# XuyangBai/D3Feat

Hardware: AMD Instinct MI355X
Metric: fragments/sec (30k-pt clouds) (higher is better)
Workload: dtype f32; 1 GPU; SURVEY §8d config #2: synthetic 3DMatch room fragment, 300k raw pts -> grid subsample 0.03 m (~29k pts per cloud) -> self-pair -> 5-level pyramid -> full KPFCNN forward (random-init weights (reference initialiser, seed 42), 14.1M params)...; points_per_cloud=29369, fragments_per_gpu=2141, parallelism=fragment-dp1, fragments_per_replay=12, engine_fallbacks=0, engine_isolated_replays=0

## Files before the change

### d3feat_amd/csrc/grid_subsample.hip

```cpp
#include <cstdlib>
#include "prims.h"
#include "radix_sort.h"

#define GS_EMPTY 0xFFFFFFFFFFFFFFFFull
#define GS_KEYBITS 56
#define GS_KEYMASK ((1ull << GS_KEYBITS) - 1ull)
#define GS_MAX_PROBE 4096

__constant__ unsigned long long D3F_CHAIN_DEV[D3F_NCHAIN] = {
    13ull, 29ull, 59ull, 127ull, 257ull, 541ull, 1109ull, 2357ull, 5087ull, 10273ull, 20753ull, 42043ull, 85229ull,
    172933ull, 351061ull, 712697ull, 1447153ull, 2938679ull, 5967347ull, 12117689ull, 24607243ull, 49969847ull,
    101473717ull, 206062531ull, 418451333ull, 849749479ull, 1725587117ull, 3504151727ull};

struct GsElem {
    float org[3];
    int pad0;
    unsigned long long NX, NY, NZ;
    long long bbase;
};

static unsigned long long gs_chain_ge(long long n) {
    for (int j = 0; j < D3F_NCHAIN; ++j)
        if ((long long)D3F_CHAIN_HOST[j] >= n) return D3F_CHAIN_HOST[j];
    return D3F_CHAIN_HOST[D3F_NCHAIN - 1];
}

__device__ __forceinline__ unsigned long long gs_mix(unsigned long long x) {
    x ^= x >> 33; x *= 0xff51afd7ed558ccdull; x ^= x >> 33; x *= 0xc4ceb9fe1a85ec53ull; x ^= x >> 33;
    return x;
}

__device__ __forceinline__ int gs_bits(unsigned long long x) {
    int b = 0;
    while (x) { ++b; x >>= 1; }
    return b;
}
__device__ __forceinline__ void gs_prep(const unsigned* __restrict__ bbox, const int* __restrict__ offs, int B, float dl,
                                        GsElem* __restrict__ el, int* __restrict__ status, RsMeta* __restrict__ smeta,
                                        int n_cap) {
    __shared__ unsigned long long sCells[256];
    const int b = threadIdx.x;
    unsigned long long cells = 0ull;
    if (b < B) {
        GsElem e;
        e.pad0 = 0;
        const int len = offs[b + 1] - offs[b];
        if (len <= 0) {
            atomicOr(&status[1], D3F_ST_EMPTY_ELEMENT);
            e.org[0] = e.org[1] = e.org[2] = 0.f;
            e.NX = e.NY = e.NZ = 1;
        } else {
            const float inv = __fdiv_rn(1.0f, dl);
            float mx[3];
#pragma unroll
            for (int d = 0; d < 3; ++d) {
                float mn = d3f_ord2f(__hip_atomic_load(&bbox[b * 6 + d], __ATOMIC_RELAXED, __HIP_MEMORY_SCOPE_AGENT));
                mx[d] = d3f_ord2f(__hip_atomic_load(&bbox[b * 6 + 3 + d], __ATOMIC_RELAXED, __HIP_MEMORY_SCOPE_AGENT));
                e.org[d] = __fmul_rn(floorf(__fmul_rn(mn, inv)), dl);
            }
            e.NX = (unsigned long long)fmaxf(floorf(__fdiv_rn(__fsub_rn(mx[0], e.org[0]), dl)), 0.f) + 1ull;
            e.NY = (unsigned long long)fmaxf(floorf(__fdiv_rn(__fsub_rn(mx[1], e.org[1]), dl)), 0.f) + 1ull;
            e.NZ = (unsigned long long)fmaxf(floorf(__fdiv_rn(__fsub_rn(mx[2], e.org[2]), dl)), 0.f) + 1ull;
        }
        long long base = 0;
        for (int j = 0; j < b; ++j) {
            long long l = offs[j + 1] - offs[j];
            unsigned long long nb = D3F_CHAIN_DEV[D3F_NCHAIN - 1];
            for (int c = 0; c < D3F_NCHAIN; ++c)
                if ((long long)D3F_CHAIN_DEV[c] >= l) { nb = D3F_CHAIN_DEV[c]; break; }
            base += (long long)nb;
        }
        e.bbase = base;
        el[b] = e;
        const double c = (double)e.NX * (double)e.NY * (double)e.NZ;
        cells = c >= 1.8e19 ? 0xFFFFFFFFFFFFFFFFull : e.NX * e.NY * e.NZ;
    }
    if (!smeta) return;
    sCells[threadIdx.x] = cells;
    __syncthreads();
    if (threadIdx.x == 0) {
        unsigned long long mx = 1ull;
        for (int j = 0; j < B; ++j) mx = sCells[j] > mx ? sCells[j] : mx;
        int kb = gs_bits(mx - 1ull);
        if (kb < 1) kb = 1;
        const int eb = gs_bits((unsigned long long)(B - 1));
        RsMeta m;
        m.n = min(offs[B], n_cap);
        m.kb = kb;
        m.bits = kb + eb;
        if (m.bits > 32) {
            atomicOr(&status[1], D3F_ST_KEY_WIDTH);
            m.n = 0;
            m.bits = 8;
        }
        m.npass = (m.bits + 7) / 8;
        *smeta = m;
    }
}
struct GsPrepEpi {
    const unsigned* bbox; const int* offs; int B; float dl; GsElem* el; int* status; RsMeta* smeta; int n_cap;
    __device__ __forceinline__ void operator()() const { gs_prep(bbox, offs, B, dl, el, status, smeta, n_cap); }
};

__global__ void __launch_bounds__(256) gs_insert_kernel(const float* __restrict__ pts, int N, const int* __restrict__ offs,
                                                        int B, float dl, const GsElem* __restrict__ el,
                                                        unsigned long long* __restrict__ tkey, unsigned* __restrict__ tfirst,
                                                        unsigned long long capmask, int* __restrict__ slot,
                                                        int* __restrict__ status) {
    const int i = blockIdx.x * blockDim.x + threadIdx.x;
    if (i >= min(N, offs[B])) return;
    const int b = d3f_find_elem(offs, B, i);
    const GsElem e = el[b];
    const float fx = floorf(__fdiv_rn(__fsub_rn(pts[3 * (size_t)i + 0], e.org[0]), dl));
    const float fy = floorf(__fdiv_rn(__fsub_rn(pts[3 * (size_t)i + 1], e.org[1]), dl));
    const float fz = floorf(__fdiv_rn(__fsub_rn(pts[3 * (size_t)i + 2], e.org[2]), dl));
    int st = 0;
    if (fx < 0.f || fy < 0.f || fz < 0.f) st |= D3F_ST_NEG_CELL;
    const unsigned long long ix = (unsigned long long)fmaxf(fx, 0.f), iy = (unsigned long long)fmaxf(fy, 0.f),
                             iz = (unsigned long long)fmaxf(fz, 0.f);
    const unsigned long long key = ix + e.NX * iy + e.NX * e.NY * iz;
    if (key > GS_KEYMASK) st |= D3F_ST_KEY_RANGE;
    if (st) atomicOr(&status[1], st);
    const unsigned long long word = ((unsigned long long)b << GS_KEYBITS) | (key & GS_KEYMASK);
    unsigned long long h = gs_mix(word) & capmask;
    bool placed = false;
    for (int probe = 0; probe < GS_MAX_PROBE; ++probe) {
        unsigned long long prev = atomicCAS(&tkey[h], GS_EMPTY, word);
        if (prev == GS_EMPTY || prev == word) { placed = true; break; }
        h = (h + 1) & capmask;
    }
    if (!placed) atomicOr(&status[1], D3F_ST_OUT_OVERFLOW);
    atomicMin(&tfirst[h], (unsigned)i);
    slot[i] = (int)h;
}

struct GsMarkIn {
    const int* n_dev; const int* slot; const unsigned* tfirst;
    __device__ __forceinline__ int operator()(int i) const { return (i < *n_dev && tfirst[slot[i]] == (unsigned)i) ? 1 : 0; }
};

__global__ void __launch_bounds__(256) gs_chain_kernel(int N, const int* __restrict__ slot, const unsigned* __restrict__ tfirst,
                                                       const unsigned long long* __restrict__ tkey,
                                                       const int* __restrict__ vscan, const int* __restrict__ vbase,
                                                       int* __restrict__ pvid,
                                                       unsigned long long* __restrict__ vkey, int* __restrict__ vhead,
                                                       int* __restrict__ vcnt, int* __restrict__ pnext,
                                                       const int* __restrict__ n_dev) {
    const int i = blockIdx.x * blockDim.x + threadIdx.x;
    if (i >= min(N, *n_dev)) return;
    const int s = slot[i];
    const int fi = (int)tfirst[s];
    const int v = d3f_scan_at(vscan, vbase, fi);
    pvid[i] = v;
    if (fi == i) vkey[v] = tkey[s] & GS_KEYMASK;
    pnext[i] = atomicExch(&vhead[v], i);
    atomicAdd(&vcnt[v], 1);
}

struct GsRankScan {
    const int* vscan; const int* vbase;
    __device__ __forceinline__ int operator()(int p) const { return d3f_scan_at(vscan, vbase, p); }
};
struct GsRankBits {
    const unsigned* fbits; const int* wscan; const int* wbase;
    __device__ __forceinline__ int operator()(int p) const {
        const int w = p >> 5;
        return d3f_scan_at(wscan, wbase, w) + __popc(fbits[w] & ((1u << (p & 31)) - 1u));
    }
};
template <class Rank>
struct GsMoffsEpi {
    const int* offs; int B; Rank rank; int* meta; int* moffs; int* sub_lens; int* status_dev;
    int out_cap;
    int elem_cap;
    __device__ __forceinline__ void operator()(int M) const {
        if (threadIdx.x != 0) return;
        meta[0] = M;
        const int N = offs[B];
        for (int b = 0; b <= B; ++b) moffs[b] = (b == B || offs[b] >= N) ? M : rank(offs[b]);
        bool over = M > out_cap ||
                    (__hip_atomic_load(&meta[1], __ATOMIC_RELAXED, __HIP_MEMORY_SCOPE_AGENT) & (D3F_ST_OUT_OVERFLOW | D3F_ST_KEY_WIDTH));
        for (int b = 0; b < B; ++b) over = over || (moffs[b + 1] - moffs[b] > elem_cap);
        if (over && !(__hip_atomic_load(&meta[1], __ATOMIC_RELAXED, __HIP_MEMORY_SCOPE_AGENT) & D3F_ST_KEY_WIDTH))
            atomicOr(&meta[1], D3F_ST_OUT_OVERFLOW);
        for (int b = 0; b < B; ++b) {
            const int l = over ? 0 : moffs[b + 1] - moffs[b];
            meta[2 + b] = l;
            sub_lens[b] = l;
        }
        if (status_dev) {
            status_dev[0] = over ? 0 : M;
            status_dev[1] = __hip_atomic_load(&meta[1], __ATOMIC_RELAXED, __HIP_MEMORY_SCOPE_AGENT);
        }
    }
};

__global__ void __launch_bounds__(256) gs_rank_kernel(int N, const int* __restrict__ n_dev, const int* __restrict__ pvid,
                                                      const int* __restrict__ vhead, const int* __restrict__ pnext,
                                                      const int* __restrict__ vstart, const int* __restrict__ sbase,
                                                      int* __restrict__ sorted) {
    const int i = blockIdx.x * blockDim.x + threadIdx.x;
    if (i >= min(N, *n_dev)) return;
    const int v = pvid[i];
    int r = 0;
    for (int j = vhead[v]; j >= 0; j = pnext[j]) r += (j < i) ? 1 : 0;
    sorted[d3f_scan_at(vstart, sbase, v) + r] = i;
}

__device__ __forceinline__ int gs_ld(const int* p) {
    return __hip_atomic_load(p, __ATOMIC_RELAXED, __HIP_MEMORY_SCOPE_AGENT);
}

__device__ __forceinline__ int gs_mod(unsigned long long key, unsigned nb, double inv_nb) {
    const unsigned long long q = (unsigned long long)((double)key * inv_nb);
    long long r = (long long)(key - q * (unsigned long long)nb);
    r += (r < 0) ? (long long)nb : 0;
    r += (r < 0) ? (long long)nb : 0;
    r -= (r >= (long long)nb) ? (long long)nb : 0;
    r -= (r >= (long long)nb) ? (long long)nb : 0;
    return (int)r;
}

#define GS_SMALL_LAST 6
#define GS_TILE 1024

struct GsOrderArgs {
    const unsigned long long* vkey;
    const int* moffs;
    const int* offs;
    const GsElem* el;
    int* P[2];
    int* nx[2];
    int* cd;
    int* bkt[2];
    int* bf[2];
    int* bc[2];
    int* bh[2];
    int* tsum;
    int* vpos;
    int max_m;
};

#define GS_SMALL_NB 1109
#define GS_SMALL_T 256
__global__ void __launch_bounds__(GS_SMALL_T) gs_order_small_kernel(GsOrderArgs A, int small_last) {
    __shared__ int wsum[GS_SMALL_T / 64];
    __shared__ int sBF[GS_SMALL_NB], sBC[GS_SMALL_NB], sBH[GS_SMALL_NB], sNX[GS_SMALL_NB], sCD[GS_SMALL_NB], sBK[GS_SMALL_NB];
    __shared__ int sL[2][GS_SMALL_NB];
    __shared__ unsigned long long sKey[GS_SMALL_NB];
    const int b = blockIdx.x;
    const int tid = threadIdx.x, lane = tid & 63, w = tid >> 6;
    const int M = A.moffs[b + 1] - A.moffs[b];
    if (M <= 0) return;
    const unsigned long long* key = A.vkey + A.moffs[b];
    int* VP = A.vpos + A.moffs[b];
    const long long bbase = A.el[b].bbase;
    if (small_last > GS_SMALL_LAST) small_last = GS_SMALL_LAST;
    for (int t = tid; t < min(M, GS_SMALL_NB); t += GS_SMALL_T) sKey[t] = key[t];
    int lo = 0, cur = 0;
    bool done = false;
    __syncthreads();
    for (int j = 0; j <= small_last && j < D3F_NCHAIN; ++j) {
        const int nb = (int)D3F_CHAIN_DEV[j];
        const double inv_nb = 1.0 / (double)nb;
        const bool last = M <= nb;
        const int hi = last ? M : nb;
        const int* La = sL[cur];
        int* Lb = sL[cur ^ 1];
        for (int t = tid; t < nb; t += GS_SMALL_T) { sBF[t] = 0x7fffffff; sBC[t] = 0; sBH[t] = -1; }
        __syncthreads();
        for (int t = tid; t < hi; t += GS_SMALL_T) {
            const int id = (t < lo) ? La[t] : t;
            const int bk = gs_mod(sKey[id], (unsigned)nb, inv_nb);
            atomicMin(&sBF[bk], t);
            atomicAdd(&sBC[bk], 1);
            sNX[t] = atomicExch(&sBH[bk], t);
            sBK[t] = bk;
        }
        __syncthreads();
        int carry = 0;
        for (int c0 = 0; c0 < hi; c0 += GS_SMALL_T) {
            const int u = c0 + tid, t = hi - 1 - u;
            int c = 0;
            if (u < hi) {
                const int bk = sBK[t];
                c = (sBF[bk] == t) ? sBC[bk] : 0;
            }
            int x = c;
#pragma unroll
            for (int d = 1; d < 64; d <<= 1) {
                int y = __shfl_up(x, d, 64);
                if (lane >= d) x += y;
            }
            if (lane == 63) wsum[w] = x;
            __syncthreads();
            int wbase = 0, tot = 0;
#pragma unroll
            for (int q = 0; q < GS_SMALL_T / 64; ++q) {
                int v = wsum[q];
                if (q < w) wbase += v;
                tot += v;
            }
            __syncthreads();
            if (u < hi) sCD[t] = carry + wbase + x - c;
            carry += tot;
        }
        __syncthreads();
        for (int t = tid; t < hi; t += GS_SMALL_T) {
            const int id = (t < lo) ? La[t] : t;
            const int bk = sBK[t];
            int r = 0;
            for (int q = sBH[bk]; q >= 0; q = sNX[q]) r += (q > t) ? 1 : 0;
            const int dest = sCD[sBF[bk]] + r;
            Lb[dest] = id;
            if (last) VP[id] = dest;
        }
        __syncthreads();
        cur ^= 1;
        if (last) { done = true; break; }
        lo = hi;
    }
    if (!done && small_last + 1 < D3F_NCHAIN) {
        const int j = small_last + 1;
        int* P = A.P[j & 1] + A.offs[b];
        for (int t = tid; t < lo; t += GS_SMALL_T) P[t] = sL[cur][t];
        const int nb = (int)D3F_CHAIN_DEV[j];
        int* BF = A.bf[j & 1] + bbase;
        int* BC = A.bc[j & 1] + bbase;
        int* BH = A.bh[j & 1] + bbase;
        for (int t = tid; t < nb; t += GS_SMALL_T) { BF[t] = 0x7fffffff; BC[t] = 0; BH[t] = -1; }
    }
}

__device__ __forceinline__ bool gs_round(const GsOrderArgs& A, int b, int j, int& M, int& lo, int& hi, int& nb, bool& last) {
    M = A.moffs[b + 1] - A.moffs[b];
    lo = (int)D3F_CHAIN_DEV[j - 1];
    if (M <= lo || M > A.max_m) return false;
    nb = (int)D3F_CHAIN_DEV[j];
    last = M <= nb;
    hi = last ? M : nb;
    return true;
}

__global__ void __launch_bounds__(256) gs_order_insert_kernel(GsOrderArgs A, int j) {
    const int b = blockIdx.y;
    int M, lo, hi, nb;
    bool last;
    if (!gs_round(A, b, j, M, lo, hi, nb, last)) return;
    const int t = blockIdx.x * 256 + threadIdx.x;
    if (t >= hi) return;
    const int o = A.offs[b];
    const long long bbase = A.el[b].bbase;
    const int id = (t < lo) ? A.P[j & 1][o + t] : t;
    const int bk = gs_mod(A.vkey[A.moffs[b] + id], (unsigned)nb, 1.0 / (double)nb);
    atomicMin(&A.bf[j & 1][bbase + bk], t);
    atomicAdd(&A.bc[j & 1][bbase + bk], 1);
    A.nx[j & 1][o + t] = atomicExch(&A.bh[j & 1][bbase + bk], t);
    A.bkt[j & 1][o + t] = bk;
}

__device__ __forceinline__ void gs_order_scan_sums(const GsOrderArgs& A, int j, int b, int* wsum) {
    int M, lo, hi, nb;
    bool last;
    if (!gs_round(A, b, j, M, lo, hi, nb, last)) return;
    int* ts = A.tsum + A.offs[b] / GS_TILE + b;
    const int ntiles = (hi + GS_TILE - 1) / GS_TILE;
    const int tid = threadIdx.x, lane = tid & 63, w = tid >> 6;
    int carry = 0;
    for (int c0 = 0; c0 < ntiles; c0 += 256) {
        const int i = c0 + tid;
        const int v = (i < ntiles) ? __hip_atomic_load(&ts[i], __ATOMIC_RELAXED, __HIP_MEMORY_SCOPE_AGENT) : 0;
        int x = v;
#pragma unroll
        for (int d = 1; d < 64; d <<= 1) {
            int y = __shfl_up(x, d, 64);
            if (lane >= d) x += y;
        }
        if (lane == 63) wsum[w] = x;
        __syncthreads();
        int wbase = 0, tot = 0;
#pragma unroll
        for (int q = 0; q < 4; ++q) {
            int s = wsum[q];
            if (q < w) wbase += s;
            tot += s;
        }
        __syncthreads();
        if (i < ntiles) ts[i] = carry + wbase + x - v;
        carry += tot;
    }
}

__global__ void __launch_bounds__(256) gs_order_scan_tiles_kernel(GsOrderArgs A, int j, int B, unsigned* __restrict__ counter) {
    __shared__ int wsum[4];
    const int b = blockIdx.y;
    int M, lo, hi, nb;
    bool last;
    const int tile = blockIdx.x;
    const bool active = gs_round(A, b, j, M, lo, hi, nb, last) && tile * GS_TILE < hi;
    if (!active) return;
    {
        const int o = A.offs[b];
        const long long bbase = A.el[b].bbase;
        const int tid = threadIdx.x, lane = tid & 63, w = tid >> 6;
        if (!last && j + 1 < D3F_NCHAIN) {
            const int nbn = (int)D3F_CHAIN_DEV[j + 1];
            const int stride = ((hi + GS_TILE - 1) / GS_TILE) * 256;
            for (int i = tile * 256 + tid; i < nbn; i += stride) {
                A.bf[(j + 1) & 1][bbase + i] = 0x7fffffff;
                A.bc[(j + 1) & 1][bbase + i] = 0;
                A.bh[(j + 1) & 1][bbase + i] = -1;
            }
        }
        int c[4], s = 0;
#pragma unroll
        for (int k = 0; k < 4; ++k) {
            const int u = tile * GS_TILE + tid * 4 + k, t = hi - 1 - u;
            c[k] = 0;
            if (u < hi) {
                const int bk = A.bkt[j & 1][o + t];
                c[k] = (A.bf[j & 1][bbase + bk] == t) ? A.bc[j & 1][bbase + bk] : 0;
            }
            s += c[k];
        }
        int x = s;
#pragma unroll
        for (int d = 1; d < 64; d <<= 1) {
            int y = __shfl_up(x, d, 64);
            if (lane >= d) x += y;
        }
        if (lane == 63) wsum[w] = x;
        __syncthreads();
        int wbase = 0, tot = 0;
#pragma unroll
        for (int q = 0; q < 4; ++q) {
            int v = wsum[q];
            if (q < w) wbase += v;
            tot += v;
        }
        int run = wbase + x - s;
#pragma unroll
        for (int k = 0; k < 4; ++k) {
            const int u = tile * GS_TILE + tid * 4 + k;
            if (u < hi) A.cd[o + hi - 1 - u] = run;
            run += c[k];
        }
        if (tid == 0) A.tsum[o / GS_TILE + b + tile] = tot;
    }
    if (!d3f_last_block(counter + b, (unsigned)((hi + GS_TILE - 1) / GS_TILE))) return;
    gs_order_scan_sums(A, j, b, wsum);
}

__global__ void __launch_bounds__(256) gs_order_place_kernel(GsOrderArgs A, int j) {
    const int b = blockIdx.y;
    int M, lo, hi, nb;
    bool last;
    if (!gs_round(A, b, j, M, lo, hi, nb, last)) return;
    const int t = blockIdx.x * 256 + threadIdx.x;
    const int o = A.offs[b];
    const long long bbase = A.el[b].bbase;
    const bool next = !last && j + 1 < D3F_NCHAIN;
    const int nbn = next ? (int)D3F_CHAIN_DEV[j + 1] : 1;
    int id = -1, pos = -1;
    if (t < hi) {
        id = (t < lo) ? A.P[j & 1][o + t] : t;
        const int bk = A.bkt[j & 1][o + t];
        int r = 0;
        for (int q = A.bh[j & 1][bbase + bk]; q >= 0; q = A.nx[j & 1][o + q]) r += (q > t) ? 1 : 0;
        const int f = A.bf[j & 1][bbase + bk];
        const int dest = A.cd[o + f] + A.tsum[o / GS_TILE + b + (hi - 1 - f) / GS_TILE] + r;
        A.P[(j + 1) & 1][o + dest] = id;
        if (last) A.vpos[A.moffs[b] + id] = dest;
        pos = dest;
    } else if (next && t < min(M, nbn)) {
        id = pos = t;
    }
    if (next && id >= 0) {
        const int bk = gs_mod(A.vkey[A.moffs[b] + id], (unsigned)nbn, 1.0 / (double)nbn);
        atomicMin(&A.bf[(j + 1) & 1][bbase + bk], pos);
        atomicAdd(&A.bc[(j + 1) & 1][bbase + bk], 1);
        A.nx[(j + 1) & 1][o + pos] = atomicExch(&A.bh[(j + 1) & 1][bbase + bk], pos);
        A.bkt[(j + 1) & 1][o + pos] = bk;
    }
}

#include "gs_small.h"

__global__ void __launch_bounds__(RS_THREADS) gs_sortkey_kernel(const float* __restrict__ pts, const float* const* __restrict__ ptrs,
                                                                const int* __restrict__ offs, int B,
                                                                float dl, const GsElem* __restrict__ el,
                                                                const RsMeta* __restrict__ smeta, unsigned* __restrict__ skey,
                                                                unsigned* __restrict__ hist, int* __restrict__ status) {
    __shared__ unsigned sHist[256];
    __shared__ int sOffs[D3F_MAX_BATCH + 1];
    __shared__ GsElem sEl[D3F_MAX_BATCH];
    __shared__ const float* sBase[D3F_MAX_BATCH];
    const int n = smeta->n, kb = smeta->kb;
    const int tile = blockIdx.x;
    if ((long long)tile * RS_TILE >= (long long)n) return;
    for (int t = threadIdx.x; t <= B; t += RS_THREADS) sOffs[t] = offs[t];
    for (int t = threadIdx.x; t < B; t += RS_THREADS) {
        sEl[t] = el[t];
        sBase[t] = ptrs ? ptrs[t] - 3 * (size_t)offs[t] : pts;
    }
    __syncthreads();
    const int w = threadIdx.x >> 6, lane = threadIdx.x & 63;
    const int base = tile * RS_TILE + w * RS_WAVE_ITEMS + lane;
    const int wlo = tile * RS_TILE + w * RS_WAVE_ITEMS, whi = min(wlo + RS_WAVE_ITEMS, n) - 1;
    int b0 = 0;
    while (b0 + 1 < B && wlo >= sOffs[b0 + 1]) ++b0;
    const bool one_cloud = (b0 + 1 >= B) || whi < sOffs[b0 + 1];
    unsigned key[RS_ROUNDS], vm = 0u;
    int st = 0;
#pragma unroll
    for (int r = 0; r < RS_ROUNDS; ++r) {
        const int i = base + r * 64;
        key[r] = 0u;
        if (i < n) {
            int b = b0;
            if (!one_cloud)
                while (b + 1 < B && i >= sOffs[b + 1]) ++b;
            const float ox = sEl[b].org[0], oy = sEl[b].org[1], oz = sEl[b].org[2];
            const unsigned NX = (unsigned)sEl[b].NX, NY = (unsigned)sEl[b].NY;
            const float* __restrict__ P = sBase[b];
            const float fx = floorf(__fdiv_rn(__fsub_rn(P[3 * (size_t)i + 0], ox), dl));
            const float fy = floorf(__fdiv_rn(__fsub_rn(P[3 * (size_t)i + 1], oy), dl));
            const float fz = floorf(__fdiv_rn(__fsub_rn(P[3 * (size_t)i + 2], oz), dl));
            if (fx < 0.f || fy < 0.f || fz < 0.f) st |= D3F_ST_NEG_CELL;
            const unsigned ix = (unsigned)fmaxf(fx, 0.f), iy = (unsigned)fmaxf(fy, 0.f), iz = (unsigned)fmaxf(fz, 0.f);
            const unsigned k = ix + NX * (iy + NY * iz);
            key[r] = (kb < 32 ? ((unsigned)b << kb) : 0u) | (kb < 32 ? (k & ((1u << kb) - 1u)) : k);
            skey[i] = key[r];
            vm |= 1u << r;
        }
    }
    if (st) atomicOr(&status[1], st);
    rs_tile_histogram(key, vm, 0, sHist, hist + (size_t)tile * 256);
}

__global__ void __launch_bounds__(256) gs_heads_kernel(int N, const RsMeta* __restrict__ smeta, const unsigned* __restrict__ key0,
                                                       const unsigned* __restrict__ key1, const unsigned* __restrict__ val0,
                                                       const unsigned* __restrict__ val1, unsigned* __restrict__ fbits) {
    const int j = blockIdx.x * blockDim.x + threadIdx.x;
    if (j >= min(N, smeta->n)) return;
    const unsigned* __restrict__ ks = (smeta->npass & 1) ? key1 : key0;
    const unsigned* __restrict__ vs = (smeta->npass & 1) ? val1 : val0;
    const unsigned k = ks[j];
    if (j == 0 || ks[j - 1] != k) {
        const unsigned i = vs[j];
        atomicOr(&fbits[i >> 5], 1u << (i & 31u));
    }
}
struct GsBitsIn {
    const unsigned* fbits;
    __device__ __forceinline__ int operator()(int w) const { return __popc(fbits[w]); }
};
__global__ void __launch_bounds__(256) gs_runs_kernel(int N, const RsMeta* __restrict__ smeta, const unsigned* __restrict__ key0,
                                                      const unsigned* __restrict__ key1, const unsigned* __restrict__ val0,
                                                      const unsigned* __restrict__ val1, GsRankBits rank,
                                                      const float* __restrict__ pts, const float* const* __restrict__ ptrs,
                                                      const int* __restrict__ offs, unsigned long long* __restrict__ vkey,
                                                      float* __restrict__ bary) {
    __shared__ float sx[256], sy[256], sz[256];
    __shared__ unsigned sk[256];
    const int n = min(N, smeta->n);
    const int j0 = blockIdx.x * 256;
    if (j0 >= n) return;
    const int t = threadIdx.x, j = j0 + t;
    const unsigned* __restrict__ ks = (smeta->npass & 1) ? key1 : key0;
    const unsigned* __restrict__ vs = (smeta->npass & 1) ? val1 : val0;
    unsigned k = 0u, pi = 0u, kprev = 0u;
    float px = 0.f, py = 0.f, pz = 0.f;
    if (j < n) {
        k = ks[j];
        pi = vs[j];
        kprev = j > 0 ? ks[j - 1] : 0u;
        if (ptrs) {
            const int b = smeta->kb < 32 ? (int)(k >> smeta->kb) : 0;
            pts = ptrs[b] - 3 * (size_t)offs[b];
        }
        px = pts[3 * (size_t)pi + 0]; py = pts[3 * (size_t)pi + 1]; pz = pts[3 * (size_t)pi + 2];
    }
    sx[t] = px; sy[t] = py; sz[t] = pz;
    sk[t] = k;
    __syncthreads();
    if (j >= n || (j != 0 && kprev == k)) return;
    const int v = rank((int)pi);
    float ax = px, ay = py, az = pz;
    int c = 1;
    const int lim = min(256, n - j0);
    while (t + c < lim && sk[t + c] == k) {
        ax = __fadd_rn(ax, sx[t + c]);
        ay = __fadd_rn(ay, sy[t + c]);
        az = __fadd_rn(az, sz[t + c]);
        ++c;
    }
    if (t + c == 256) {
        while (j + c < n && ks[j + c] == k) {
            const size_t q = vs[j + c];
            ax = __fadd_rn(ax, pts[3 * q + 0]);
            ay = __fadd_rn(ay, pts[3 * q + 1]);
            az = __fadd_rn(az, pts[3 * q + 2]);
            ++c;
        }
    }
    const float sc = (float)(1.0 / (double)c);
    vkey[v] = (unsigned long long)(smeta->kb < 32 ? (k & ((1u << smeta->kb) - 1u)) : k);
    bary[3 * (size_t)v + 0] = __fmul_rn(ax, sc);
    bary[3 * (size_t)v + 1] = __fmul_rn(ay, sc);
    bary[3 * (size_t)v + 2] = __fmul_rn(az, sc);
}
__global__ void __launch_bounds__(256) gs_emit_kernel(int* __restrict__ status, const int* __restrict__ moffs, int B,
                                                      const int* __restrict__ vpos, const float* __restrict__ bary,
                                                      float* __restrict__ out_p, int out_cap) {
    const int v = blockIdx.x * blockDim.x + threadIdx.x;
    if (v >= status[0]) return;
    const int b = d3f_find_elem(moffs, B, v);
    const size_t dest = (size_t)moffs[b] + (size_t)vpos[v];
    if (dest >= (size_t)out_cap) {
        atomicOr(&status[1], D3F_ST_OUT_OVERFLOW);
        return;
    }
    out_p[3 * dest + 0] = bary[3 * (size_t)v + 0];
    out_p[3 * dest + 1] = bary[3 * (size_t)v + 1];
    out_p[3 * dest + 2] = bary[3 * (size_t)v + 2];
}


__global__ void __launch_bounds__(256) gs_accum_kernel(const float* __restrict__ pts, const float* __restrict__ feat,
                                                       int fdim, int* __restrict__ status,
                                                       const int* __restrict__ moffs, int B,
                                                       const int* __restrict__ vstart, const int* __restrict__ sbase,
                                                       const int* __restrict__ vcnt,
                                                       const int* __restrict__ sorted, const int* __restrict__ vpos,
                                                       float* __restrict__ out_p, float* __restrict__ out_f, int out_cap) {
    const int v = blockIdx.x * blockDim.x + threadIdx.x;
    if (v >= status[0]) return;
    const int b = d3f_find_elem(moffs, B, v);
    const int n = vcnt[v], st = sbase ? d3f_scan_at(vstart, sbase, v) : vstart[v];
    const size_t dest = (size_t)moffs[b] + (size_t)vpos[v];
    if (dest >= (size_t)out_cap) {
        atomicOr(&status[1], D3F_ST_OUT_OVERFLOW);
        return;
    }
    float sx = 0.f, sy = 0.f, sz = 0.f;
    for (int t = 0; t < n; ++t) {
        const size_t i = (size_t)sorted[st + t];
        sx = __fadd_rn(sx, pts[3 * i + 0]);
        sy = __fadd_rn(sy, pts[3 * i + 1]);
        sz = __fadd_rn(sz, pts[3 * i + 2]);
    }
    const float sc = (float)(1.0 / (double)n);
    out_p[3 * dest + 0] = __fmul_rn(sx, sc);
    out_p[3 * dest + 1] = __fmul_rn(sy, sc);
    out_p[3 * dest + 2] = __fmul_rn(sz, sc);
    if (fdim > 0) {
        const float cf = (float)n;
        for (int f = 0; f < fdim; ++f) {
            float s = 0.f;
            for (int t = 0; t < n; ++t) s = __fadd_rn(s, feat[(size_t)sorted[st + t] * fdim + f]);
            out_f[dest * fdim + f] = __fdiv_rn(s, cf);
        }
    }
}

__global__ void __launch_bounds__(256) gs_fill_kernel(int* __restrict__ p, size_t n, int v) {
    const size_t i = (size_t)blockIdx.x * blockDim.x + threadIdx.x;
    if (i < n) p[i] = v;
}
__global__ void __launch_bounds__(256) gs_labels_kernel(int N, int ldim, const int* __restrict__ cls,
                                                        const int* __restrict__ pvid, const int* __restrict__ moffs, int B,
                                                        const int* __restrict__ vpos, int* __restrict__ out_c) {
    const int i = blockIdx.x * blockDim.x + threadIdx.x;
    if (i >= N) return;
    const int v = pvid[i];
    const int b = d3f_find_elem(moffs, B, v);
    const size_t dest = (size_t)moffs[b] + (size_t)vpos[v];
    for (int l = 0; l < ldim; ++l) atomicMax(&out_c[dest * ldim + l], cls[(size_t)i * ldim + l]);
}

struct GsLayout {
    size_t cap;
    long long bucket_total;
};
static GsLayout gs_layout(int N, int B, int keys = -1) {
    GsLayout L;
    L.cap = 64;
    const size_t nk = (size_t)((keys > 0 && keys < N) ? keys : (N > 0 ? N : 1));
    while (L.cap < (size_t)2 * nk) L.cap <<= 1;
    L.bucket_total = (long long)(2.24 * (double)N) + 16ll * B + 64;
    return L;
}

extern "C" size_t d3f_grid_subsample_workspace_bytes(int N, int B, int fdim, int ldim) {
    (void)fdim; (void)ldim;
    if (N < 0 || B < 1) return 0;
    GsLayout L = gs_layout(N, B);
    size_t n = (size_t)(N > 0 ? N : 1);
    size_t bytes = 0;
    bytes += d3f_align((B + 1) * sizeof(int)) * 2 + d3f_align((B + 2) * sizeof(int));
    bytes += d3f_align(B * 6 * sizeof(unsigned));
    bytes += d3f_align(B * sizeof(GsElem));
    bytes += d3f_align(L.cap * sizeof(unsigned long long));
    bytes += d3f_align(L.cap * sizeof(int));
    bytes += d3f_align(n * sizeof(unsigned long long));
    bytes += 16 * d3f_align(n * sizeof(int));
    bytes += 6 * d3f_align((size_t)L.bucket_total * sizeof(int));
    bytes += d3f_align((n / GS_TILE + B + 8) * sizeof(int));
    bytes += 2 * d3f_align(d3f_scan_base_ints(N) * sizeof(int)) + d3f_align((4 + D3F_NCHAIN * (size_t)B) * sizeof(unsigned));
    bytes += d3f_align(rs_hist_words(N) * sizeof(unsigned)) + d3f_align((n / 32 + 2) * sizeof(unsigned)) +
             d3f_align(3 * n * sizeof(float)) + d3f_align(sizeof(RsMeta));
    bytes += d3f_align(7 * (size_t)B * (n < 16384 ? n : 16384) * sizeof(float)) + 256 + 2 * d3f_align(B * sizeof(int));
    return bytes + 4096;
}

template <int T, int R>
static int gs_small_launch(const GsSmallArgs& A, float* sub_points, int* sub_lens_dev, int* status_dev, hipStream_t stream) {
    static std::atomic<unsigned long long> lds_done{0ull};
    const void* const fns[] = {(const void*)gs_small_kernel<T, R>};
    if (d3f_opt_in_lds(lds_done, fns, (int)gss_lds_bytes<T, R>(GSS_NB_MAX)) != D3F_OK) return D3F_ERR_HIP;
    gs_small_kernel<T, R><<<A.B, T, gss_lds_bytes<T, R>(A.nbmax), stream>>>(A);
    D3F_LAUNCH_CHECK();
    gs_small_pack_kernel<<<d3f_cdiv(A.out_cap, 256), 256, 0, stream>>>(A, sub_points, sub_lens_dev, status_dev);
    D3F_LAUNCH_CHECK();
    return D3F_OK;
}
static int gs_run_small(const float* points, int N, const int* lens_dev, int B, float dl, float* sub_points, int M_cap, int elem_cap,
                        int pc, int* sub_lens_dev, int* status_dev, void* workspace, size_t workspace_bytes, hipStream_t stream) {
    if (elem_cap <= 0 || elem_cap > M_cap) elem_cap = M_cap;
    if (elem_cap > pc) elem_cap = pc;
    D3fArena ar(workspace, workspace_bytes);
    GsSmallArgs A;
    A.stage = ar.take<float>(3 * (size_t)B * (size_t)elem_cap);
    A.recs = ar.take<float>(4 * (size_t)B * (size_t)elem_cap);
    A.mcount = ar.take<int>(B);
    A.cflags = ar.take<int>(B);
    if (!ar.ok) return D3F_ERR_WORKSPACE;
    A.pts = points; A.lens = lens_dev; A.B = B; A.dl = dl; A.elem_cap = elem_cap; A.out_cap = M_cap;
    A.nbmax = GSS_NB_MAX;
    for (int j = 0; j < D3F_NCHAIN; ++j)
        if ((long long)D3F_CHAIN_HOST[j] >= (long long)elem_cap) { A.nbmax = (int)D3F_CHAIN_HOST[j]; break; }
    if (A.nbmax > GSS_NB_MAX) A.nbmax = GSS_NB_MAX;
    if (A.nbmax < 1109) A.nbmax = 1109;
    if (pc <= 2048) return gs_small_launch<256, 8>(A, sub_points, sub_lens_dev, status_dev, stream);
    if (pc <= 4096) return gs_small_launch<512, 8>(A, sub_points, sub_lens_dev, status_dev, stream);
    if (pc <= 8192) return gs_small_launch<1024, 8>(A, sub_points, sub_lens_dev, status_dev, stream);
    if (pc <= 12288) return gs_small_launch<1024, 12>(A, sub_points, sub_lens_dev, status_dev, stream);
    return gs_small_launch<1024, 16>(A, sub_points, sub_lens_dev, status_dev, stream);
}

static int gs_run(const float* points, int N, const int* lens_dev, int B, float dl, const float* features, int fdim,
                  const int* classes, int ldim, float* sub_points, int M_cap, int elem_cap, int elem_points, float* sub_features,
                  int* sub_classes, int* sub_lens_dev, int* status_host, int* status_dev, void* workspace,
                  size_t workspace_bytes, hipStream_t stream, const float* const* ptrs = nullptr) {
    const bool async = status_dev != nullptr;
    if (async && !features && ldim == 0 && !ptrs) {
        const int pc = (elem_points > 0 && elem_points < N) ? elem_points : N;
        int ec = (elem_cap > 0 && elem_cap < M_cap) ? elem_cap : M_cap;
        if (ec > pc) ec = pc;
        if (pc <= 16384 && ec <= GSS_NB_MAX) return gs_run_small(points, N, lens_dev, B, dl, sub_points, M_cap, elem_cap, pc, sub_lens_dev, status_dev,
                                             workspace, workspace_bytes, stream);
    }
    GsLayout L = gs_layout(N, B, async ? M_cap : -1);
    D3fArena ar(workspace, workspace_bytes);
    const size_t n = (size_t)N;
    int* offs = ar.take<int>(B + 1);
    int* moffs = ar.take<int>(B + 1);
    unsigned* bbox = ar.take<unsigned>(B * 6);
    GsElem* el = ar.take<GsElem>(B);
    const int ncounters = 4 + D3F_NCHAIN * B;
    unsigned* counters = ar.take<unsigned>(ncounters);
    unsigned long long* tkey = ar.take<unsigned long long>(L.cap);
    unsigned* tfirst = ar.take<unsigned>(L.cap);
    int* vhead = ar.take<int>(n);
    int* meta = ar.take<int>(B + 2);
    int* vcnt = ar.take<int>(n);
    unsigned long long* vkey = ar.take<unsigned long long>(n);
    int* slot = ar.take<int>(n);
    int* vscan = ar.take<int>(n);
    int* pvid = ar.take<int>(n);
    int* pnext = ar.take<int>(n);
    int* vstart = ar.take<int>(n);
    int* sorted = ar.take<int>(n);
    GsOrderArgs A;
    A.vpos = ar.take<int>(n);
    A.P[0] = ar.take<int>(n);
    A.P[1] = ar.take<int>(n);
    A.nx[0] = ar.take<int>(n);
    A.nx[1] = ar.take<int>(n);
    A.cd = ar.take<int>(n);
    A.bkt[0] = ar.take<int>(n);
    A.bkt[1] = ar.take<int>(n);
    for (int k = 0; k < 2; ++k) {
        A.bf[k] = ar.take<int>((size_t)L.bucket_total);
        A.bc[k] = ar.take<int>((size_t)L.bucket_total);
        A.bh[k] = ar.take<int>((size_t)L.bucket_total);
    }
    A.tsum = ar.take<int>(n / GS_TILE + B + 8);
    int* vbase = ar.take<int>(d3f_scan_base_ints(N));
    int* sbase = ar.take<int>(d3f_scan_base_ints(N));
    const bool use_sort = async && !features && ldim == 0;
    unsigned* rs_hist = ar.take<unsigned>(rs_hist_words(N));
    unsigned* fbits = ar.take<unsigned>(n / 32 + 2);
    float* bary = ar.take<float>(3 * n);
    RsMeta* smeta = ar.take<RsMeta>(1);
    if (!ar.ok) return D3F_ERR_WORKSPACE;
    A.vkey = vkey; A.moffs = moffs; A.offs = offs; A.el = el;
    if (elem_cap <= 0 || elem_cap > M_cap) elem_cap = M_cap;
    if (elem_cap > N) elem_cap = N;
    A.max_m = async ? elem_cap : 0x7fffffff;

    int rc;
    const D3fFill none{nullptr, 0ull, 0u};
    const unsigned long long ones_words = (unsigned long long)((char*)(vhead + n) - (char*)tkey) / 4ull;
    const unsigned long long zero_words = (unsigned long long)((char*)(vcnt + n) - (char*)meta) / 4ull;
    if ((rc = use_sort ? d3f_begin_launch(lens_dev, B, offs, bbox, counters, ncounters, D3fFill{fbits, (unsigned long long)(n / 32 + 2), 0u},
                                          D3fFill{(unsigned*)meta, (unsigned long long)(B + 2), 0u}, none, none, stream)
                       : d3f_begin_launch(lens_dev, B, offs, bbox, counters, ncounters, D3fFill{(unsigned*)tkey, ones_words, 0xFFFFFFFFu},
                                          D3fFill{(unsigned*)meta, zero_words, 0u}, none, none, stream)) != D3F_OK) return rc;
    GsPrepEpi prep{bbox, offs, B, dl, el, meta, use_sort ? smeta : nullptr, N};
    if ((rc = d3f_bbox_launch_t(points, offs, B, N, bbox, counters, prep, stream, ptrs)) != D3F_OK) return rc;
    const int nblk = d3f_cdiv(N, 256);
    const int elem_lim = async ? elem_cap : 0x7fffffff;
    int M, maxM;
    if (use_sort) {
        unsigned *key0 = (unsigned*)slot, *key1 = (unsigned*)pnext, *val0 = (unsigned*)pvid, *val1 = (unsigned*)sorted;
        gs_sortkey_kernel<<<rs_tiles(N), RS_THREADS, 0, stream>>>(points, ptrs, offs, B, dl, el, smeta, key0, rs_hist, meta);
        D3F_LAUNCH_CHECK();
        if ((rc = rs_sort_launch(smeta, N, key0, key1, val0, val1, rs_hist, stream)) != D3F_OK) return rc;
        gs_heads_kernel<<<nblk, 256, 0, stream>>>(N, smeta, key0, key1, val0, val1, fbits);
        D3F_LAUNCH_CHECK();
        const GsRankBits rank{fbits, vscan, vbase};
        GsMoffsEpi<GsRankBits> mepi{offs, B, rank, meta, moffs, sub_lens_dev, status_dev, M_cap, elem_lim};
        if ((rc = d3f_scan_fold_launch(GsBitsIn{fbits}, N / 32 + 1, nullptr, vscan, vbase, counters + 1, mepi, stream)) != D3F_OK)
            return rc;
        gs_runs_kernel<<<nblk, 256, 0, stream>>>(N, smeta, key0, key1, val0, val1, rank, points, ptrs, offs, vkey, bary);
        D3F_LAUNCH_CHECK();
        M = N < M_cap ? N : M_cap;
        maxM = elem_cap;
    } else {
    GsMoffsEpi<GsRankScan> mepi{offs, B, GsRankScan{vscan, vbase}, meta, moffs, sub_lens_dev, status_dev, M_cap, elem_lim};
    gs_insert_kernel<<<nblk, 256, 0, stream>>>(points, N, offs, B, dl, el, tkey, tfirst, (unsigned long long)L.cap - 1ull,
                                               slot, meta);
    D3F_LAUNCH_CHECK();
    if ((rc = d3f_scan_fold_launch(GsMarkIn{offs + B, slot, tfirst}, N, offs + B, vscan, vbase, counters + 1, mepi, stream)) != D3F_OK)
        return rc;
    if (!async) {
        D3F_HIP_TRY(hipMemcpyAsync(status_host, meta, (B + 2) * sizeof(int), hipMemcpyDeviceToHost, stream));
        D3F_HIP_TRY(hipStreamSynchronize(stream));
        M = status_host[0];
        if (status_host[1] != 0 || M <= 0) return D3F_OK;
        maxM = 0;
        for (int b = 0; b < B; ++b) maxM = status_host[2 + b] > maxM ? status_host[2 + b] : maxM;
    } else {
        M = N < M_cap ? N : M_cap;
        maxM = elem_cap;
    }

    gs_chain_kernel<<<nblk, 256, 0, stream>>>(N, slot, tfirst, tkey, vscan, vbase, pvid, vkey, vhead, vcnt, pnext, offs + B);
    D3F_LAUNCH_CHECK();
    if ((rc = d3f_scan_fold_launch(D3fScanIn{vcnt}, async ? N : M, meta, vstart, sbase, counters + 2, D3fNoEpi{}, stream)) != D3F_OK)
        return rc;
    gs_rank_kernel<<<nblk, 256, 0, stream>>>(N, offs + B, pvid, vhead, pnext, vstart, sbase, sorted);
    }
    const int small_last = GS_SMALL_LAST;
    gs_order_small_kernel<<<B, GS_SMALL_T, 0, stream>>>(A, small_last);
    for (int j = small_last + 1; j < D3F_NCHAIN && (long long)D3F_CHAIN_HOST[j - 1] < (long long)maxM; ++j) {
        const long long nbj = (long long)D3F_CHAIN_HOST[j];
        const int hi = (int)((long long)maxM < nbj ? (long long)maxM : nbj);
        const bool more = j + 1 < D3F_NCHAIN && nbj < (long long)maxM;
        const long long nbn = more ? (long long)D3F_CHAIN_HOST[j + 1] : 0;
        const int hin = more ? (int)((long long)maxM < nbn ? (long long)maxM : nbn) : hi;
        dim3 g(d3f_cdiv(hi, 256), B), gt(d3f_cdiv(hi, GS_TILE), B), gp(d3f_cdiv(hin > hi ? hin : hi, 256), B);
        if (j == small_last + 1) gs_order_insert_kernel<<<g, 256, 0, stream>>>(A, j);
        gs_order_scan_tiles_kernel<<<gt, 256, 0, stream>>>(A, j, B, counters + 4 + j * B);
        gs_order_place_kernel<<<gp, 256, 0, stream>>>(A, j);
    }
    if (use_sort)
        gs_emit_kernel<<<d3f_cdiv(M, 256), 256, 0, stream>>>(meta, moffs, B, A.vpos, bary, sub_points, M_cap);
    else
        gs_accum_kernel<<<d3f_cdiv(async ? N : M, 256), 256, 0, stream>>>(points, features, fdim, meta, moffs, B, vstart, sbase,
                                                                         vcnt, sorted, A.vpos, sub_points, sub_features, M_cap);
    if (ldim > 0) {
        const size_t tot = (size_t)M * (size_t)ldim;
        gs_fill_kernel<<<d3f_cdiv((long long)tot, 256), 256, 0, stream>>>(sub_classes, tot, (int)0x80000000);
        gs_labels_kernel<<<nblk, 256, 0, stream>>>(N, ldim, classes, pvid, moffs, B, A.vpos, sub_classes);
    }
    D3F_LAUNCH_CHECK();
    return D3F_OK;
}

extern "C" int d3f_batch_grid_subsample(const float* points, int N, const int* lens_dev, int B, float dl,
                                        const float* features, int fdim, const int* classes, int ldim,
                                        float* sub_points, float* sub_features, int* sub_classes, int* sub_lens_dev,
                                        int* status_host, void* workspace, size_t workspace_bytes, void* stream_) {
    hipStream_t stream = (hipStream_t)stream_;
    if (N < 0 || N > (1 << 30) || B < 1 || B > D3F_MAX_BATCH || !(dl > 0.f) || fdim < 0 || ldim < 0) return D3F_ERR_ARG;
    if (!points || !lens_dev || !sub_points || !sub_lens_dev || !status_host) return D3F_ERR_ARG;
    if ((fdim > 0 && (!features || !sub_features)) || (ldim > 0 && (!classes || !sub_classes))) return D3F_ERR_ARG;
    for (int i = 0; i < B + 2; ++i) status_host[i] = 0;
    if (N == 0) return d3f_fill_u32(sub_lens_dev, B, 0u, stream);
    return gs_run(points, N, lens_dev, B, dl, features, fdim, classes, ldim, sub_points, N, N, 0, sub_features, sub_classes,
                  sub_lens_dev, status_host, nullptr, workspace, workspace_bytes, stream);
}

extern "C" int d3f_batch_grid_subsample_async(const float* points, int N_cap, const int* lens_dev, int B, float dl,
                                              float* sub_points, int M_cap, int elem_cap, int elem_points_cap, int* sub_lens_dev,
                                              int* status_dev, void* workspace, size_t workspace_bytes, void* stream_) {
    hipStream_t stream = (hipStream_t)stream_;
    if (N_cap < 1 || N_cap > (1 << 30) || M_cap < 1 || elem_cap < 0 || elem_points_cap < 0 || B < 1 || B > D3F_MAX_BATCH || !(dl > 0.f))
        return D3F_ERR_ARG;
    if (!points || !lens_dev || !sub_points || !sub_lens_dev || !status_dev) return D3F_ERR_ARG;
    return gs_run(points, N_cap, lens_dev, B, dl, nullptr, 0, nullptr, 0, sub_points, M_cap, elem_cap, elem_points_cap, nullptr,
                  nullptr, sub_lens_dev, nullptr, status_dev, workspace, workspace_bytes, stream);
}

extern "C" int d3f_batch_grid_subsample_async_inplace(const float* const* clouds_dev, int N_cap, const int* lens_dev, int B, float dl,
                                                      float* sub_points, int M_cap, int elem_cap, int* sub_lens_dev, int* status_dev,
                                                      void* workspace, size_t workspace_bytes, void* stream_) {
    hipStream_t stream = (hipStream_t)stream_;
    if (N_cap < 1 || N_cap > (1 << 30) || M_cap < 1 || elem_cap < 0 || B < 1 || B > D3F_MAX_BATCH || !(dl > 0.f)) return D3F_ERR_ARG;
    if (!clouds_dev || !lens_dev || !sub_points || !sub_lens_dev || !status_dev) return D3F_ERR_ARG;
    return gs_run(nullptr, N_cap, lens_dev, B, dl, nullptr, 0, nullptr, 0, sub_points, M_cap, elem_cap, 0, nullptr, nullptr, sub_lens_dev,
                  nullptr, status_dev, workspace, workspace_bytes, stream, clouds_dev);
}

__global__ void __launch_bounds__(256) gs_stack_pair_kernel(const float* __restrict__ pts, int M_cap, const int* __restrict__ lens_in,
                                                            int B, float* __restrict__ out, int* __restrict__ lens_out,
                                                            int* __restrict__ total) {
    const int i = blockIdx.x * blockDim.x + threadIdx.x;
    int tot = 0;
    for (int b = 0; b < B; ++b) tot += lens_in[b];
    tot = min(tot, M_cap);
    if (i == 0) {
        int room = M_cap;
        for (int b = 0; b < B; ++b) {
            const int m = min(lens_in[b], room);
            room -= m;
            lens_out[2 * b] = m;
            lens_out[2 * b + 1] = m;
        }
        *total = 2 * tot;
    }
    if (i >= 3 * tot) return;
    const int pi = i / 3, c = i - 3 * pi;
    int start = 0, m = 0;
    for (int b = 0; b < B; ++b) {
        m = lens_in[b];
        if (pi < start + m || b == B - 1) break;
        start += m;
    }
    m = min(m, tot - start);
    const float v = pts[i];
    const size_t row = 2 * (size_t)start + (size_t)(pi - start);
    out[3 * row + c] = v;
    out[3 * (row + m) + c] = v;
}

extern "C" int d3f_stack_self_pair(const float* pts, int M_cap, const int* lens_in_dev, int B, float* out, int* lens_out_dev,
                                   int* total_dev, void* stream_) {
    hipStream_t stream = (hipStream_t)stream_;
    if (M_cap < 1 || B < 1 || 2 * B > D3F_MAX_BATCH || !pts || !lens_in_dev || !out || !lens_out_dev || !total_dev)
        return D3F_ERR_ARG;
    gs_stack_pair_kernel<<<d3f_cdiv(3ll * M_cap, 256), 256, 0, stream>>>(pts, M_cap, lens_in_dev, B, out, lens_out_dev, total_dev);
    D3F_LAUNCH_CHECK();
    return D3F_OK;
}
```

### d3feat_amd/csrc/radix_sort.h

```cpp
#pragma once
#include "common.h"

#define RS_THREADS 512
#define RS_WAVES (RS_THREADS / 64)
#define RS_ROUNDS 16
#define RS_TILE (RS_THREADS * RS_ROUNDS)
#define RS_WAVE_ITEMS (64 * RS_ROUNDS)
#define RS_MAX_PASSES 4

struct RsMeta {
    int n;
    int bits;
    int npass;
    int kb;
};

#define RS_SCATTER_LDS_BYTES ((2 * RS_WAVES * 256 + 256 + 16 + 2 * RS_TILE) * 4)
static inline int rs_tiles(int n_cap) { return d3f_cdiv(n_cap > 0 ? n_cap : 1, RS_TILE); }
static inline size_t rs_hist_words(int n_cap) { return (size_t)rs_tiles(n_cap) * 256; }

#ifdef __HIPCC__
__device__ __forceinline__ void rs_tile_histogram(const unsigned (&key)[RS_ROUNDS], unsigned valid_mask, int shift,
                                                  unsigned* __restrict__ sHist, unsigned* __restrict__ hist_row) {
    if (threadIdx.x < 256) sHist[threadIdx.x] = 0u;
    __syncthreads();
#pragma unroll
    for (int r = 0; r < RS_ROUNDS; ++r)
        if (valid_mask & (1u << r)) atomicAdd(&sHist[(key[r] >> shift) & 255u], 1u);
    __syncthreads();
    if (threadIdx.x < 256) hist_row[threadIdx.x] = sHist[threadIdx.x];
}

__global__ void __launch_bounds__(RS_THREADS) rs_hist_kernel(const RsMeta* __restrict__ meta, int pass,
                                                             const unsigned* __restrict__ key0,
                                                             const unsigned* __restrict__ key1,
                                                             unsigned* __restrict__ hist) {
    __shared__ unsigned sHist[256];
    const int n = meta->n;
    if (pass >= meta->npass) return;
    const int tile = blockIdx.x;
    if ((long long)tile * RS_TILE >= (long long)n) return;
    const unsigned* __restrict__ src = (pass & 1) ? key1 : key0;
    const int w = threadIdx.x >> 6, lane = threadIdx.x & 63;
    const int base = tile * RS_TILE + w * RS_WAVE_ITEMS + lane;
    unsigned key[RS_ROUNDS], vm = 0u;
#pragma unroll
    for (int r = 0; r < RS_ROUNDS; ++r) {
        const int pos = base + r * 64;
        key[r] = 0u;
        if (pos < n) { key[r] = src[pos]; vm |= 1u << r; }
    }
    rs_tile_histogram(key, vm, pass * 8, sHist, hist + (size_t)tile * 256);
}

__global__ void __launch_bounds__(RS_THREADS) rs_scatter_kernel(const RsMeta* __restrict__ meta, int pass,
                                                                unsigned* __restrict__ key0, unsigned* __restrict__ key1,
                                                                unsigned* __restrict__ val0, unsigned* __restrict__ val1,
                                                                const unsigned* __restrict__ hist) {
    extern __shared__ __attribute__((aligned(16))) unsigned rs_lds[];
    unsigned (*sCnt)[256] = (unsigned (*)[256])rs_lds;
    unsigned (*sPart)[256] = (unsigned (*)[256])(rs_lds + RS_WAVES * 256);
    unsigned* sBase = rs_lds + 2 * RS_WAVES * 256;
    unsigned* sScan = sBase + 256;
    unsigned* sKey = sScan + 16;
    unsigned* sVal = sKey + RS_TILE;
    const int n = meta->n;
    if (pass >= meta->npass) return;
    const int tile = blockIdx.x;
    if ((long long)tile * RS_TILE >= (long long)n) return;
    const int live = (n + RS_TILE - 1) / RS_TILE;
    const unsigned* __restrict__ ksrc = (pass & 1) ? key1 : key0;
    const unsigned* __restrict__ vsrc = (pass & 1) ? val1 : val0;
    unsigned* __restrict__ kdst = (pass & 1) ? key0 : key1;
    unsigned* __restrict__ vdst = (pass & 1) ? val0 : val1;
    const int tid = threadIdx.x, w = tid >> 6, lane = tid & 63;
    const int shift = pass * 8;

    const int base = tile * RS_TILE + w * RS_WAVE_ITEMS + lane;
    unsigned key[RS_ROUNDS], val[RS_ROUNDS];
#pragma unroll
    for (int r = 0; r < RS_ROUNDS; ++r) {
        const int pos = base + r * 64;
        key[r] = 0u;
        val[r] = (unsigned)pos;
        if (pos < n) {
            key[r] = ksrc[pos];
            if (pass > 0) val[r] = vsrc[pos];
        }
    }
    {
        uint4 bef = make_uint4(0u, 0u, 0u, 0u), tot = make_uint4(0u, 0u, 0u, 0u);
        const uint4* __restrict__ rows = (const uint4*)hist + lane;
        int t = w;
        for (; t + 7 * RS_WAVES < live; t += 8 * RS_WAVES) {
            uint4 v[8];
#pragma unroll
            for (int u = 0; u < 8; ++u) v[u] = rows[(size_t)(t + u * RS_WAVES) * 64];
#pragma unroll
            for (int u = 0; u < 8; ++u) {
                tot.x += v[u].x; tot.y += v[u].y; tot.z += v[u].z; tot.w += v[u].w;
                if (t + u * RS_WAVES < tile) { bef.x += v[u].x; bef.y += v[u].y; bef.z += v[u].z; bef.w += v[u].w; }
            }
        }
        for (; t < live; t += RS_WAVES) {
            const uint4 v = rows[(size_t)t * 64];
            tot.x += v.x; tot.y += v.y; tot.z += v.z; tot.w += v.w;
            if (t < tile) { bef.x += v.x; bef.y += v.y; bef.z += v.z; bef.w += v.w; }
        }
        ((uint4*)sCnt[w])[lane] = tot;
        ((uint4*)sPart[w])[lane] = bef;
    }
    __syncthreads();
    {
        unsigned total = 0u, before = 0u;
        if (tid < 256) {
#pragma unroll
            for (int q = 0; q < RS_WAVES; ++q) { total += sCnt[q][tid]; before += sPart[q][tid]; }
        }
        unsigned x = total;
#pragma unroll
        for (int d = 1; d < 64; d <<= 1) {
            const unsigned y = (unsigned)__shfl_up((int)x, d, 64);
            if (lane >= d) x += y;
        }
        if (lane == 63) sScan[w] = x;
        __syncthreads();
#pragma unroll
        for (int q = 0; q < RS_WAVES; ++q)
            if (tid < 256) sCnt[q][tid] = 0u;
        unsigned wb = 0u;
#pragma unroll
        for (int q = 0; q < 4; ++q) wb += (q < w) ? sScan[q] : 0u;
        if (tid < 256) sBase[tid] = wb + x - total + before;
        __syncthreads();
    }
    unsigned rank[RS_ROUNDS];
    volatile unsigned* myCnt = sCnt[w];
#pragma unroll
    for (int r = 0; r < RS_ROUNDS; ++r) {
        const bool valid = (base + r * 64) < n;
        const unsigned dg = (key[r] >> shift) & 255u;
        unsigned long long peers = __ballot(valid);
#pragma unroll
        for (int bit = 0; bit < 8; ++bit) {
            const bool one = (dg >> bit) & 1u;
            const unsigned long long m = __ballot(one);
            peers &= one ? m : ~m;
        }
        rank[r] = 0u;
        if (valid) {
            const unsigned prev = myCnt[dg];
            const unsigned below = (unsigned)__popcll(peers & d3f_lanemask_lt());
            rank[r] = prev + below;
            __builtin_amdgcn_wave_barrier();
            if (below == 0u) myCnt[dg] = prev + (unsigned)__popcll(peers);
        }
        __builtin_amdgcn_wave_barrier();
    }
    __syncthreads();
    {
        unsigned cnt = 0u;
        if (tid < 256) {
#pragma unroll
            for (int q = 0; q < RS_WAVES; ++q) cnt += sCnt[q][tid];
        }
        unsigned x = cnt;
#pragma unroll
        for (int d = 1; d < 64; d <<= 1) {
            const unsigned y = (unsigned)__shfl_up((int)x, d, 64);
            if (lane >= d) x += y;
        }
        if (lane == 63) sScan[w] = x;
        __syncthreads();
        if (tid < 256) {
            unsigned wb = 0u;
#pragma unroll
            for (int q = 0; q < 4; ++q) wb += (q < w) ? sScan[q] : 0u;
            const unsigned loc = wb + x - cnt;
            unsigned run = loc;
#pragma unroll
            for (int q = 0; q < RS_WAVES; ++q) {
                const unsigned c = sCnt[q][tid];
                sCnt[q][tid] = run;
                run += c;
            }
            sBase[tid] -= loc;
        }
    }
    __syncthreads();
#pragma unroll
    for (int r = 0; r < RS_ROUNDS; ++r) {
        if ((base + r * 64) < n) {
            const unsigned dg = (key[r] >> shift) & 255u;
            const unsigned pl = myCnt[dg] + rank[r];
            sKey[pl] = key[r];
            sVal[pl] = val[r];
        }
    }
    __syncthreads();
    const int tile_n = min(RS_TILE, n - tile * RS_TILE);
#pragma unroll
    for (int r = 0; r < RS_ROUNDS; ++r) {
        const int pl = r * RS_THREADS + tid;
        if (pl < tile_n) {
            const unsigned k = sKey[pl];
            const unsigned dest = sBase[(k >> shift) & 255u] + (unsigned)pl;
            kdst[dest] = k;
            vdst[dest] = sVal[pl];
        }
    }
}
#endif

static inline int rs_sort_launch(const RsMeta* meta, int n_cap, unsigned* key0, unsigned* key1, unsigned* val0, unsigned* val1,
                                 unsigned* hist, hipStream_t stream) {
    const int tiles = rs_tiles(n_cap);
    static std::atomic<unsigned long long> lds_done{0ull};
    const void* const fns[] = {(const void*)rs_scatter_kernel};
    if (d3f_opt_in_lds(lds_done, fns, RS_SCATTER_LDS_BYTES) != D3F_OK) return D3F_ERR_HIP;
    for (int p = 0; p < RS_MAX_PASSES; ++p) {
        if (p > 0) {
            rs_hist_kernel<<<tiles, RS_THREADS, 0, stream>>>(meta, p, key0, key1, hist);
            D3F_LAUNCH_CHECK();
        }
        rs_scatter_kernel<<<tiles, RS_THREADS, RS_SCATTER_LDS_BYTES, stream>>>(meta, p, key0, key1, val0, val1, hist);
        D3F_LAUNCH_CHECK();
    }
    return D3F_OK;
}
```

Before: 1865 fragments/s.

## Fuse grid-subsample ordering rounds and radix sort into single-pass decoupled-lookback kernels

The bucket-ordering rounds now run as one kernel per round instead of separate insert, tile-scan and place kernels. Tiles are handed out by an atomic ticket and prefix sums resolve through decoupled lookback with tagged descriptors, and the bucket tables are triple-buffered so the next-next round can be cleared early. The small-block kernel also does the first large round's insert directly. The radix sort swaps its per-pass histogram kernel for global histograms of every digit computed once in the key kernel, plus per-tile lookback inside the scatter kernel. The aim is fewer launches and fewer global passes, at the cost of spin-waiting with a timeout flag, which depends on forward-progress ordering of the tickets.

New measurement: 1879 fragments/s (median of 6 runs). Within noise of the previous version (+0.7%).

```diff
diff --git a/d3feat_amd/csrc/grid_subsample.hip b/d3feat_amd/csrc/grid_subsample.hip
--- a/d3feat_amd/csrc/grid_subsample.hip
+++ b/d3feat_amd/csrc/grid_subsample.hip
@@ -222,7 +222,10 @@
 }
 
 #define GS_SMALL_LAST 6
-#define GS_TILE 1024
+#define GS_PT 256
+#define GS_AGG 1u
+#define GS_INC 2u
+#define GS_DONE 3u
 
 struct GsOrderArgs {
     const unsigned long long* vkey;
@@ -233,10 +236,11 @@
     int* nx[2];
     int* cd;
     int* bkt[2];
-    int* bf[2];
-    int* bc[2];
-    int* bh[2];
-    int* tsum;
+    int* bf[3];
+    int* bc[3];
+    int* bh[3];
+    unsigned long long* look;
+    int* flags;
     int* vpos;
     int max_m;
 };
@@ -320,15 +324,49 @@
         if (last) { done = true; break; }
         lo = hi;
     }
-    if (!done && small_last + 1 < D3F_NCHAIN) {
+    if (!done && small_last + 1 < D3F_NCHAIN && M <= A.max_m) {
         const int j = small_last + 1;
-        int* P = A.P[j & 1] + A.offs[b];
+        const int o = A.offs[b];
+        int* P = A.P[j & 1] + o;
         for (int t = tid; t < lo; t += GS_SMALL_T) P[t] = sL[cur][t];
         const int nb = (int)D3F_CHAIN_DEV[j];
-        int* BF = A.bf[j & 1] + bbase;
-        int* BC = A.bc[j & 1] + bbase;
-        int* BH = A.bh[j & 1] + bbase;
+        const int hi = M <= nb ? M : nb;
+        int* BF = A.bf[j % 3] + bbase;
+        int* BC = A.bc[j % 3] + bbase;
+        int* BH = A.bh[j % 3] + bbase;
         for (int t = tid; t < nb; t += GS_SMALL_T) { BF[t] = 0x7fffffff; BC[t] = 0; BH[t] = -1; }
+        asm volatile("s_waitcnt vmcnt(0)" ::: "memory");
+        __syncthreads();
+        if (M > nb && j + 1 < D3F_NCHAIN) {
+            const int nbn = (int)D3F_CHAIN_DEV[j + 1], s = (j + 1) % 3;
+            for (int t = tid; t < nbn; t += GS_SMALL_T) { A.bf[s][bbase + t] = 0x7fffffff; A.bc[s][bbase + t] = 0; A.bh[s][bbase + t] = -1; }
+        }
+        int* NX = A.nx[j & 1] + o;
+        int* BK = A.bkt[j & 1] + o;
+        const double inv_nb = 1.0 / (double)nb;
+        for (int t0 = tid; t0 < hi; t0 += 4 * GS_SMALL_T) {
+            int bk[4], prev[4];
+#pragma unroll
+            for (int u = 0; u < 4; ++u) {
+                const int t = t0 + u * GS_SMALL_T;
+                bk[u] = t < hi ? gs_mod(key[(t < lo) ? sL[cur][t] : t], (unsigned)nb, inv_nb) : -1;
+            }
+#pragma unroll
+            for (int u = 0; u < 4; ++u) {
+                const int t = t0 + u * GS_SMALL_T;
+                prev[u] = -1;
+                if (bk[u] >= 0) {
+                    atomicMin(&BF[bk[u]], t);
+                    atomicAdd(&BC[bk[u]], 1);
+                    prev[u] = atomicExch(&BH[bk[u]], t);
+                }
+            }
+#pragma unroll
+            for (int u = 0; u < 4; ++u) {
+                const int t = t0 + u * GS_SMALL_T;
+                if (bk[u] >= 0) { NX[t] = prev[u]; BK[t] = bk[u]; }
+            }
+        }
     }
 }
 
@@ -342,38 +380,66 @@
     return true;
 }
 
-__global__ void __launch_bounds__(256) gs_order_insert_kernel(GsOrderArgs A, int j) {
+#define GS_SPIN_LIMIT (1u << 20)
+__device__ __forceinline__ unsigned long long gs_word(unsigned tag, int v) {
+    return ((unsigned long long)tag << 32) | (unsigned)v;
+}
+__device__ __forceinline__ unsigned long long gs_poll(const unsigned long long* p, int j, unsigned kmin, int* flags) {
+    for (unsigned spins = 0;; ++spins) {
+        const unsigned long long v = __hip_atomic_load(p, __ATOMIC_RELAXED, __HIP_MEMORY_SCOPE_AGENT);
+        const unsigned tag = (unsigned)(v >> 32);
+        if (tag >= 4u * j + kmin && tag <= 4u * j + GS_DONE) return v;
+        if (spins >= GS_SPIN_LIMIT) {
+            atomicOr(flags, D3F_ST_OUT_OVERFLOW);
+            return gs_word(4u * j + GS_DONE, 0);
+        }
+        __builtin_amdgcn_s_sleep(1);
+    }
+}
+
+__global__ void __launch_bounds__(256) gs_order_round_kernel(GsOrderArgs A, int j, unsigned* __restrict__ counter) {
+    __shared__ int wsum[4];
+    __shared__ int sP[GS_PT];
+    __shared__ int sTile, sExcl;
     const int b = blockIdx.y;
     int M, lo, hi, nb;
     bool last;
     if (!gs_round(A, b, j, M, lo, hi, nb, last)) return;
-    const int t = blockIdx.x * 256 + threadIdx.x;
-    if (t >= hi) return;
+    const int tid = threadIdx.x, lane = tid & 63, w = tid >> 6;
     const int o = A.offs[b];
     const long long bbase = A.el[b].bbase;
-    const int id = (t < lo) ? A.P[j & 1][o + t] : t;
-    const int bk = gs_mod(A.vkey[A.moffs[b] + id], (unsigned)nb, 1.0 / (double)nb);
-    atomicMin(&A.bf[j & 1][bbase + bk], t);
-    atomicAdd(&A.bc[j & 1][bbase + bk], 1);
-    A.nx[j & 1][o + t] = atomicExch(&A.bh[j & 1][bbase + bk], t);
-    A.bkt[j & 1][o + t] = bk;
-}
-
-__device__ __forceinline__ void gs_order_scan_sums(const GsOrderArgs& A, int j, int b, int* wsum) {
-    int M, lo, hi, nb;
-    bool last;
-    if (!gs_round(A, b, j, M, lo, hi, nb, last)) return;
-    int* ts = A.tsum + A.offs[b] / GS_TILE + b;
-    const int ntiles = (hi + GS_TILE - 1) / GS_TILE;
-    const int tid = threadIdx.x, lane = tid & 63, w = tid >> 6;
-    int carry = 0;
-    for (int c0 = 0; c0 < ntiles; c0 += 256) {
-        const int i = c0 + tid;
-        const int v = (i < ntiles) ? __hip_atomic_load(&ts[i], __ATOMIC_RELAXED, __HIP_MEMORY_SCOPE_AGENT) : 0;
-        int x = v;
+    const bool next = !last && j + 1 < D3F_NCHAIN;
+    const int nbn = next ? (int)D3F_CHAIN_DEV[j + 1] : 1;
+    if (next && j + 2 < D3F_NCHAIN && M > nbn) {
+        const int nb2 = (int)D3F_CHAIN_DEV[j + 2], s = (j + 2) % 3;
+        for (int i = blockIdx.x * GS_PT + tid; i < nb2; i += gridDim.x * GS_PT) {
+            A.bf[s][bbase + i] = 0x7fffffff;
+            A.bc[s][bbase + i] = 0;
+            A.bh[s][bbase + i] = -1;
+        }
+    }
+    const int cs = j % 3;
+    const int ntiles = (hi + GS_PT - 1) / GS_PT;
+    int tile = blockIdx.x;
+    if ((int)blockIdx.x < ntiles) {
+        if (tid == 0) sTile = (int)atomicAdd(counter + b, 1u);
+        __syncthreads();
+        tile = sTile;
+    }
+    const int t = tile * GS_PT + tid;
+    int id = -1, pos = -1;
+    if (tile < ntiles) {
+        unsigned long long* L = A.look + o / GS_PT + b;
+        int bk = 0, f = 0, c = 0;
+        if (t < hi) {
+            bk = A.bkt[j & 1][o + t];
+            f = A.bf[cs][bbase + bk];
+            c = (f == t) ? A.bc[cs][bbase + bk] : 0;
+        }
+        int x = c;
 #pragma unroll
         for (int d = 1; d < 64; d <<= 1) {
-            int y = __shfl_up(x, d, 64);
+            const int y = __shfl_up(x, d, 64);
             if (lane >= d) x += y;
         }
         if (lane == 63) wsum[w] = x;
@@ -381,105 +447,82 @@
         int wbase = 0, tot = 0;
 #pragma unroll
         for (int q = 0; q < 4; ++q) {
-            int s = wsum[q];
-            if (q < w) wbase += s;
-            tot += s;
-        }
-        __syncthreads();
-        if (i < ntiles) ts[i] = carry + wbase + x - v;
-        carry += tot;
-    }
-}
-
-__global__ void __launch_bounds__(256) gs_order_scan_tiles_kernel(GsOrderArgs A, int j, int B, unsigned* __restrict__ counter) {
-    __shared__ int wsum[4];
-    const int b = blockIdx.y;
-    int M, lo, hi, nb;
-    bool last;
-    const int tile = blockIdx.x;
-    const bool active = gs_round(A, b, j, M, lo, hi, nb, last) && tile * GS_TILE < hi;
-    if (!active) return;
-    {
-        const int o = A.offs[b];
-        const long long bbase = A.el[b].bbase;
-        const int tid = threadIdx.x, lane = tid & 63, w = tid >> 6;
-        if (!last && j + 1 < D3F_NCHAIN) {
-            const int nbn = (int)D3F_CHAIN_DEV[j + 1];
-            const int stride = ((hi + GS_TILE - 1) / GS_TILE) * 256;
-            for (int i = tile * 256 + tid; i < nbn; i += stride) {
-                A.bf[(j + 1) & 1][bbase + i] = 0x7fffffff;
-                A.bc[(j + 1) & 1][bbase + i] = 0;
-                A.bh[(j + 1) & 1][bbase + i] = -1;
-            }
-        }
-        int c[4], s = 0;
-#pragma unroll
-        for (int k = 0; k < 4; ++k) {
-            const int u = tile * GS_TILE + tid * 4 + k, t = hi - 1 - u;
-            c[k] = 0;
-            if (u < hi) {
-                const int bk = A.bkt[j & 1][o + t];
-                c[k] = (A.bf[j & 1][bbase + bk] == t) ? A.bc[j & 1][bbase + bk] : 0;
-            }
-            s += c[k];
-        }
-        int x = s;
-#pragma unroll
-        for (int d = 1; d < 64; d <<= 1) {
-            int y = __shfl_up(x, d, 64);
-            if (lane >= d) x += y;
-        }
-        if (lane == 63) wsum[w] = x;
-        __syncthreads();
-        int wbase = 0, tot = 0;
-#pragma unroll
-        for (int q = 0; q < 4; ++q) {
-            int v = wsum[q];
+            const int v = wsum[q];
             if (q < w) wbase += v;
             tot += v;
         }
-        int run = wbase + x - s;
+        if (w == 0) {
+            if (lane == 0)
+                __hip_atomic_store(L + tile, gs_word(4u * j + (tile == 0 ? GS_INC : GS_AGG), tot), __ATOMIC_RELAXED,
+                                   __HIP_MEMORY_SCOPE_AGENT);
+            int ex = 0;
+            for (int k = tile - 1, spins = 0; k >= 0;) {
+                const unsigned long long v = (k - lane >= 0) ? __hip_atomic_load(L + k - lane, __ATOMIC_RELAXED, __HIP_MEMORY_SCOPE_AGENT)
+                                                             : gs_word(4u * j + GS_INC, 0);
+                const unsigned tag = (unsigned)(v >> 32);
+                const bool ready = tag >= 4u * j + GS_AGG && tag <= 4u * j + GS_DONE;
+                const unsigned long long nr = __ballot(!ready), im = __ballot(ready && tag >= 4u * j + GS_INC);
+                const int fnr = nr ? __ffsll((long long)nr) - 1 : 64, finc = im ? __ffsll((long long)im) - 1 : 64;
+                const int take = finc < fnr ? finc + 1 : fnr;
+                int sum = lane < take ? (int)(unsigned)v : 0;
 #pragma unroll
-        for (int k = 0; k < 4; ++k) {
-            const int u = tile * GS_TILE + tid * 4 + k;
-            if (u < hi) A.cd[o + hi - 1 - u] = run;
-            run += c[k];
-        }
-        if (tid == 0) A.tsum[o / GS_TILE + b + tile] = tot;
-    }
-    if (!d3f_last_block(counter + b, (unsigned)((hi + GS_TILE - 1) / GS_TILE))) return;
-    gs_order_scan_sums(A, j, b, wsum);
-}
-
-__global__ void __launch_bounds__(256) gs_order_place_kernel(GsOrderArgs A, int j) {
-    const int b = blockIdx.y;
-    int M, lo, hi, nb;
-    bool last;
-    if (!gs_round(A, b, j, M, lo, hi, nb, last)) return;
-    const int t = blockIdx.x * 256 + threadIdx.x;
-    const int o = A.offs[b];
-    const long long bbase = A.el[b].bbase;
-    const bool next = !last && j + 1 < D3F_NCHAIN;
-    const int nbn = next ? (int)D3F_CHAIN_DEV[j + 1] : 1;
-    int id = -1, pos = -1;
-    if (t < hi) {
-        id = (t < lo) ? A.P[j & 1][o + t] : t;
-        const int bk = A.bkt[j & 1][o + t];
-        int r = 0;
-        for (int q = A.bh[j & 1][bbase + bk]; q >= 0; q = A.nx[j & 1][o + q]) r += (q > t) ? 1 : 0;
-        const int f = A.bf[j & 1][bbase + bk];
-        const int dest = A.cd[o + f] + A.tsum[o / GS_TILE + b + (hi - 1 - f) / GS_TILE] + r;
-        A.P[(j + 1) & 1][o + dest] = id;
-        if (last) A.vpos[A.moffs[b] + id] = dest;
-        pos = dest;
+                for (int o = 32; o > 0; o >>= 1) sum += __shfl_xor(sum, o, 64);
+                ex += sum;
+                if (finc < fnr) break;
+                k -= take;
+                if (take == 0) {
+                    if (++spins >= (int)GS_SPIN_LIMIT) {
+                        if (lane == 0) atomicOr(A.flags, D3F_ST_OUT_OVERFLOW);
+                        break;
+                    }
+                    __builtin_amdgcn_s_sleep(1);
+                }
+            }
+            if (lane == 0) {
+                if (tile > 0)
+                    __hip_atomic_store(L + tile, gs_word(4u * j + GS_INC, ex + tot), __ATOMIC_RELAXED, __HIP_MEMORY_SCOPE_AGENT);
+                sExcl = ex;
+            }
+        }
+        __syncthreads();
+        const int pt = sExcl + wbase + x;
+        sP[tid] = pt;
+        if (t < hi) __hip_atomic_store(&A.cd[o + t], pt, __ATOMIC_RELAXED, __HIP_MEMORY_SCOPE_AGENT);
+        asm volatile("s_waitcnt vmcnt(0)" ::: "memory");
+        __syncthreads();
+        if (tid == 0) __hip_atomic_store(L + tile, gs_word(4u * j + GS_DONE, sExcl + tot), __ATOMIC_RELAXED, __HIP_MEMORY_SCOPE_AGENT);
+        if (t < hi) {
+            id = (t < lo) ? A.P[j & 1][o + t] : t;
+            int r = 0;
+            for (int q = A.bh[cs][bbase + bk]; q >= 0; q = A.nx[j & 1][o + q]) r += (q > t) ? 1 : 0;
+            int pf;
+            if (f >= tile * GS_PT) {
+                pf = sP[f - tile * GS_PT];
+            } else {
+                gs_poll(L + f / GS_PT, j, GS_DONE, A.flags);
+                __builtin_amdgcn_fence(__ATOMIC_ACQUIRE, "wavefront");
+                pf = __hip_atomic_load(&A.cd[o + f], __ATOMIC_RELAXED, __HIP_MEMORY_SCOPE_AGENT);
+            }
+            const int dest = hi - pf + r;
+            if ((unsigned)dest < (unsigned)hi) {
+                A.P[(j + 1) & 1][o + dest] = id;
+                if (last) A.vpos[A.moffs[b] + id] = dest;
+                pos = dest;
+            } else {
+                id = -1;
+            }
+        } else if (next && t < min(M, nbn)) {
+            id = pos = t;
+        }
     } else if (next && t < min(M, nbn)) {
         id = pos = t;
     }
     if (next && id >= 0) {
+        const int ns = (j + 1) % 3;
         const int bk = gs_mod(A.vkey[A.moffs[b] + id], (unsigned)nbn, 1.0 / (double)nbn);
-        atomicMin(&A.bf[(j + 1) & 1][bbase + bk], pos);
-        atomicAdd(&A.bc[(j + 1) & 1][bbase + bk], 1);
-        A.nx[(j + 1) & 1][o + pos] = atomicExch(&A.bh[(j + 1) & 1][bbase + bk], pos);
+        atomicMin(&A.bf[ns][bbase + bk], pos);
+        atomicAdd(&A.bc[ns][bbase + bk], 1);
+        A.nx[(j + 1) & 1][o + pos] = atomicExch(&A.bh[ns][bbase + bk], pos);
         A.bkt[(j + 1) & 1][o + pos] = bk;
     }
 }
@@ -490,8 +533,8 @@
                                                                 const int* __restrict__ offs, int B,
                                                                 float dl, const GsElem* __restrict__ el,
                                                                 const RsMeta* __restrict__ smeta, unsigned* __restrict__ skey,
-                                                                unsigned* __restrict__ hist, int* __restrict__ status) {
-    __shared__ unsigned sHist[256];
+                                                                unsigned* __restrict__ ghist, int* __restrict__ status) {
+    __shared__ unsigned sHist[RS_MAX_PASSES * 256];
     __shared__ int sOffs[D3F_MAX_BATCH + 1];
     __shared__ GsElem sEl[D3F_MAX_BATCH];
     __shared__ const float* sBase[D3F_MAX_BATCH];
@@ -535,7 +578,7 @@
         }
     }
     if (st) atomicOr(&status[1], st);
-    rs_tile_histogram(key, vm, 0, sHist, hist + (size_t)tile * 256);
+    rs_key_histograms(key, vm, smeta->npass, sHist, ghist);
 }
 
 __global__ void __launch_bounds__(256) gs_heads_kernel(int N, const RsMeta* __restrict__ smeta, const unsigned* __restrict__ key0,
@@ -705,10 +748,10 @@
     bytes += d3f_align(L.cap * sizeof(int));
     bytes += d3f_align(n * sizeof(unsigned long long));
     bytes += 16 * d3f_align(n * sizeof(int));
-    bytes += 6 * d3f_align((size_t)L.bucket_total * sizeof(int));
-    bytes += d3f_align((n / GS_TILE + B + 8) * sizeof(int));
+    bytes += 9 * d3f_align((size_t)L.bucket_total * sizeof(int));
+    bytes += d3f_align((n / GS_PT + B + 8) * sizeof(unsigned long long));
     bytes += 2 * d3f_align(d3f_scan_base_ints(N) * sizeof(int)) + d3f_align((4 + D3F_NCHAIN * (size_t)B) * sizeof(unsigned));
-    bytes += d3f_align(rs_hist_words(N) * sizeof(unsigned)) + d3f_align((n / 32 + 2) * sizeof(unsigned)) +
+    bytes += d3f_align(rs_state_words(N) * sizeof(unsigned)) + d3f_align((n / 32 + 2) * sizeof(unsigned)) +
              d3f_align(3 * n * sizeof(float)) + d3f_align(sizeof(RsMeta));
     bytes += d3f_align(7 * (size_t)B * (n < 16384 ? n : 16384) * sizeof(float)) + 256 + 2 * d3f_align(B * sizeof(int));
     return bytes + 4096;
@@ -791,21 +834,21 @@
     A.cd = ar.take<int>(n);
     A.bkt[0] = ar.take<int>(n);
     A.bkt[1] = ar.take<int>(n);
-    for (int k = 0; k < 2; ++k) {
+    for (int k = 0; k < 3; ++k) {
         A.bf[k] = ar.take<int>((size_t)L.bucket_total);
         A.bc[k] = ar.take<int>((size_t)L.bucket_total);
         A.bh[k] = ar.take<int>((size_t)L.bucket_total);
     }
-    A.tsum = ar.take<int>(n / GS_TILE + B + 8);
     int* vbase = ar.take<int>(d3f_scan_base_ints(N));
     int* sbase = ar.take<int>(d3f_scan_base_ints(N));
     const bool use_sort = async && !features && ldim == 0;
-    unsigned* rs_hist = ar.take<unsigned>(rs_hist_words(N));
+    A.look = ar.take<unsigned long long>(n / GS_PT + B + 8);
+    unsigned* rs_state = ar.take<unsigned>(rs_state_words(N));
     unsigned* fbits = ar.take<unsigned>(n / 32 + 2);
     float* bary = ar.take<float>(3 * n);
     RsMeta* smeta = ar.take<RsMeta>(1);
     if (!ar.ok) return D3F_ERR_WORKSPACE;
-    A.vkey = vkey; A.moffs = moffs; A.offs = offs; A.el = el;
+    A.vkey = vkey; A.moffs = moffs; A.offs = offs; A.el = el; A.flags = meta + 1;
     if (elem_cap <= 0 || elem_cap > M_cap) elem_cap = M_cap;
     if (elem_cap > N) elem_cap = N;
     A.max_m = async ? elem_cap : 0x7fffffff;
@@ -814,10 +857,12 @@
     const D3fFill none{nullptr, 0ull, 0u};
     const unsigned long long ones_words = (unsigned long long)((char*)(vhead + n) - (char*)tkey) / 4ull;
     const unsigned long long zero_words = (unsigned long long)((char*)(vcnt + n) - (char*)meta) / 4ull;
+    const char* look_end = use_sort ? (const char*)(rs_state + rs_state_words(N)) : (const char*)(A.look + n / GS_PT + B + 8);
+    const D3fFill look_fill{(unsigned*)A.look, (unsigned long long)(look_end - (const char*)A.look) / 4ull, 0u};
     if ((rc = use_sort ? d3f_begin_launch(lens_dev, B, offs, bbox, counters, ncounters, D3fFill{fbits, (unsigned long long)(n / 32 + 2), 0u},
-                                          D3fFill{(unsigned*)meta, (unsigned long long)(B + 2), 0u}, none, none, stream)
+                                          D3fFill{(unsigned*)meta, (unsigned long long)(B + 2), 0u}, look_fill, none, stream)
                        : d3f_begin_launch(lens_dev, B, offs, bbox, counters, ncounters, D3fFill{(unsigned*)tkey, ones_words, 0xFFFFFFFFu},
-                                          D3fFill{(unsigned*)meta, zero_words, 0u}, none, none, stream)) != D3F_OK) return rc;
+                                          D3fFill{(unsigned*)meta, zero_words, 0u}, look_fill, none, stream)) != D3F_OK) return rc;
     GsPrepEpi prep{bbox, offs, B, dl, el, meta, use_sort ? smeta : nullptr, N};
     if ((rc = d3f_bbox_launch_t(points, offs, B, N, bbox, counters, prep, stream, ptrs)) != D3F_OK) return rc;
     const int nblk = d3f_cdiv(N, 256);
@@ -825,9 +870,10 @@
     int M, maxM;
     if (use_sort) {
         unsigned *key0 = (unsigned*)slot, *key1 = (unsigned*)pnext, *val0 = (unsigned*)pvid, *val1 = (unsigned*)sorted;
-        gs_sortkey_kernel<<<rs_tiles(N), RS_THREADS, 0, stream>>>(points, ptrs, offs, B, dl, el, smeta, key0, rs_hist, meta);
+        gs_sortkey_kernel<<<rs_tiles(N), RS_THREADS, 0, stream>>>(points, ptrs, offs, B, dl, el, smeta, key0, rs_ghist(rs_state, N),
+                                                                   meta);
         D3F_LAUNCH_CHECK();
-        if ((rc = rs_sort_launch(smeta, N, key0, key1, val0, val1, rs_hist, stream)) != D3F_OK) return rc;
+        if ((rc = rs_sort_launch(smeta, N, key0, key1, val0, val1, rs_state, meta + 1, stream)) != D3F_OK) return rc;
         gs_heads_kernel<<<nblk, 256, 0, stream>>>(N, smeta, key0, key1, val0, val1, fbits);
         D3F_LAUNCH_CHECK();
         const GsRankBits rank{fbits, vscan, vbase};
@@ -871,10 +917,8 @@
         const bool more = j + 1 < D3F_NCHAIN && nbj < (long long)maxM;
         const long long nbn = more ? (long long)D3F_CHAIN_HOST[j + 1] : 0;
         const int hin = more ? (int)((long long)maxM < nbn ? (long long)maxM : nbn) : hi;
-        dim3 g(d3f_cdiv(hi, 256), B), gt(d3f_cdiv(hi, GS_TILE), B), gp(d3f_cdiv(hin > hi ? hin : hi, 256), B);
-        if (j == small_last + 1) gs_order_insert_kernel<<<g, 256, 0, stream>>>(A, j);
-        gs_order_scan_tiles_kernel<<<gt, 256, 0, stream>>>(A, j, B, counters + 4 + j * B);
-        gs_order_place_kernel<<<gp, 256, 0, stream>>>(A, j);
+        const dim3 gp(d3f_cdiv(hin > hi ? hin : hi, GS_PT), B);
+        gs_order_round_kernel<<<gp, 256, 0, stream>>>(A, j, counters + 4 + j * B);
     }
     if (use_sort)
         gs_emit_kernel<<<d3f_cdiv(M, 256), 256, 0, stream>>>(meta, moffs, B, A.vpos, bary, sub_points, M_cap);
diff --git a/d3feat_amd/csrc/radix_sort.h b/d3feat_amd/csrc/radix_sort.h
--- a/d3feat_amd/csrc/radix_sort.h
+++ b/d3feat_amd/csrc/radix_sort.h
@@ -7,6 +7,8 @@
 #define RS_TILE (RS_THREADS * RS_ROUNDS)
 #define RS_WAVE_ITEMS (64 * RS_ROUNDS)
 #define RS_MAX_PASSES 4
+#define RS_LOOK 4
+#define RS_SPIN_LIMIT (1u << 20)
 
 struct RsMeta {
     int n;
@@ -15,65 +17,67 @@
     int kb;
 };
 
-#define RS_SCATTER_LDS_BYTES ((2 * RS_WAVES * 256 + 256 + 16 + 2 * RS_TILE) * 4)
+#define RS_SCATTER_LDS_BYTES ((RS_WAVES * 256 + 256 + 16 + 2 * RS_TILE) * 4)
 static inline int rs_tiles(int n_cap) { return d3f_cdiv(n_cap > 0 ? n_cap : 1, RS_TILE); }
-static inline size_t rs_hist_words(int n_cap) { return (size_t)rs_tiles(n_cap) * 256; }
+static inline size_t rs_state_words(int n_cap) { return (size_t)rs_tiles(n_cap) * 256 + RS_MAX_PASSES * 256 + 16; }
+static inline unsigned* rs_ghist(unsigned* state, int n_cap) { return state + (size_t)rs_tiles(n_cap) * 256; }
 
 #ifdef __HIPCC__
-__device__ __forceinline__ void rs_tile_histogram(const unsigned (&key)[RS_ROUNDS], unsigned valid_mask, int shift,
-                                                  unsigned* __restrict__ sHist, unsigned* __restrict__ hist_row) {
-    if (threadIdx.x < 256) sHist[threadIdx.x] = 0u;
-    __syncthreads();
-#pragma unroll
-    for (int r = 0; r < RS_ROUNDS; ++r)
-        if (valid_mask & (1u << r)) atomicAdd(&sHist[(key[r] >> shift) & 255u], 1u);
-    __syncthreads();
-    if (threadIdx.x < 256) hist_row[threadIdx.x] = sHist[threadIdx.x];
-}
-
-__global__ void __launch_bounds__(RS_THREADS) rs_hist_kernel(const RsMeta* __restrict__ meta, int pass,
-                                                             const unsigned* __restrict__ key0,
-                                                             const unsigned* __restrict__ key1,
-                                                             unsigned* __restrict__ hist) {
-    __shared__ unsigned sHist[256];
-    const int n = meta->n;
-    if (pass >= meta->npass) return;
-    const int tile = blockIdx.x;
-    if ((long long)tile * RS_TILE >= (long long)n) return;
-    const unsigned* __restrict__ src = (pass & 1) ? key1 : key0;
-    const int w = threadIdx.x >> 6, lane = threadIdx.x & 63;
-    const int base = tile * RS_TILE + w * RS_WAVE_ITEMS + lane;
-    unsigned key[RS_ROUNDS], vm = 0u;
-#pragma unroll
-    for (int r = 0; r < RS_ROUNDS; ++r) {
-        const int pos = base + r * 64;
-        key[r] = 0u;
-        if (pos < n) { key[r] = src[pos]; vm |= 1u << r; }
-    }
-    rs_tile_histogram(key, vm, pass * 8, sHist, hist + (size_t)tile * 256);
+__device__ __forceinline__ void rs_key_histograms(const unsigned (&key)[RS_ROUNDS], unsigned valid_mask, int npass,
+                                                  unsigned* __restrict__ sHist, unsigned* __restrict__ ghist) {
+    for (int i = threadIdx.x; i < RS_MAX_PASSES * 256; i += RS_THREADS) sHist[i] = 0u;
+    __syncthreads();
+    for (int p = 0; p < npass; ++p) {
+#pragma unroll
+        for (int r = 0; r < RS_ROUNDS; ++r) {
+            const bool valid = (valid_mask >> r) & 1u;
+            const unsigned dg = (key[r] >> (8 * p)) & 255u;
+            const unsigned d0 = (unsigned)__builtin_amdgcn_readfirstlane((int)dg);
+            const unsigned long long vb = __ballot(valid);
+            if (__all(!valid || dg == d0)) {
+                if ((threadIdx.x & 63) == 0 && vb) atomicAdd(&sHist[p * 256 + d0], (unsigned)__popcll(vb));
+            } else if (valid) {
+                atomicAdd(&sHist[p * 256 + dg], 1u);
+            }
+        }
+    }
+    __syncthreads();
+    for (int i = threadIdx.x; i < npass * 256; i += RS_THREADS) {
+        const unsigned c = sHist[i];
+        if (c) atomicAdd(&ghist[i], c);
+    }
+}
+
+__device__ __forceinline__ bool rs_row_ready(const unsigned long long (&v)[2], unsigned tag) {
+    return (((unsigned)v[0] & 0xffff0000u) == tag) & (((unsigned)(v[0] >> 32) & 0xffff0000u) == tag) &
+           (((unsigned)v[1] & 0xffff0000u) == tag) & (((unsigned)(v[1] >> 32) & 0xffff0000u) == tag);
 }
 
 __global__ void __launch_bounds__(RS_THREADS) rs_scatter_kernel(const RsMeta* __restrict__ meta, int pass,
                                                                 unsigned* __restrict__ key0, unsigned* __restrict__ key1,
                                                                 unsigned* __restrict__ val0, unsigned* __restrict__ val1,
-                                                                const unsigned* __restrict__ hist) {
+                                                                unsigned* __restrict__ look,
+                                                                const unsigned* __restrict__ ghist,
+                                                                unsigned* __restrict__ tickets, int* __restrict__ flags) {
     extern __shared__ __attribute__((aligned(16))) unsigned rs_lds[];
     unsigned (*sCnt)[256] = (unsigned (*)[256])rs_lds;
-    unsigned (*sPart)[256] = (unsigned (*)[256])(rs_lds + RS_WAVES * 256);
-    unsigned* sBase = rs_lds + 2 * RS_WAVES * 256;
+    unsigned* sBase = rs_lds + RS_WAVES * 256;
     unsigned* sScan = sBase + 256;
     unsigned* sKey = sScan + 16;
     unsigned* sVal = sKey + RS_TILE;
     const int n = meta->n;
     if (pass >= meta->npass) return;
-    const int tile = blockIdx.x;
-    if ((long long)tile * RS_TILE >= (long long)n) return;
     const int live = (n + RS_TILE - 1) / RS_TILE;
+    if ((int)blockIdx.x >= live) return;
+    const int tid = threadIdx.x, w = tid >> 6, lane = tid & 63;
+    if (tid == 0) sScan[12] = atomicAdd(&tickets[pass], 1u);
+    for (int i = tid; i < RS_WAVES * 256 + 256; i += RS_THREADS) rs_lds[i] = 0u;
+    __syncthreads();
+    const int tile = (int)sScan[12];
     const unsigned* __restrict__ ksrc = (pass & 1) ? key1 : key0;
     const unsigned* __restrict__ vsrc = (pass & 1) ? val1 : val0;
     unsigned* __restrict__ kdst = (pass & 1) ? key0 : key1;
     unsigned* __restrict__ vdst = (pass & 1) ? val0 : val1;
-    const int tid = threadIdx.x, w = tid >> 6, lane = tid & 63;
     const int shift = pass * 8;
 
     const int base = tile * RS_TILE + w * RS_WAVE_ITEMS + lane;
@@ -87,52 +91,6 @@
             key[r] = ksrc[pos];
             if (pass > 0) val[r] = vsrc[pos];
         }
-    }
-    {
-        uint4 bef = make_uint4(0u, 0u, 0u, 0u), tot = make_uint4(0u, 0u, 0u, 0u);
-        const uint4* __restrict__ rows = (const uint4*)hist + lane;
-        int t = w;
-        for (; t + 7 * RS_WAVES < live; t += 8 * RS_WAVES) {
-            uint4 v[8];
-#pragma unroll
-            for (int u = 0; u < 8; ++u) v[u] = rows[(size_t)(t + u * RS_WAVES) * 64];
-#pragma unroll
-            for (int u = 0; u < 8; ++u) {
-                tot.x += v[u].x; tot.y += v[u].y; tot.z += v[u].z; tot.w += v[u].w;
-                if (t + u * RS_WAVES < tile) { bef.x += v[u].x; bef.y += v[u].y; bef.z += v[u].z; bef.w += v[u].w; }
-            }
-        }
-        for (; t < live; t += RS_WAVES) {
-            const uint4 v = rows[(size_t)t * 64];
-            tot.x += v.x; tot.y += v.y; tot.z += v.z; tot.w += v.w;
-            if (t < tile) { bef.x += v.x; bef.y += v.y; bef.z += v.z; bef.w += v.w; }
-        }
-        ((uint4*)sCnt[w])[lane] = tot;
-        ((uint4*)sPart[w])[lane] = bef;
-    }
-    __syncthreads();
-    {
-        unsigned total = 0u, before = 0u;
-        if (tid < 256) {
-#pragma unroll
-            for (int q = 0; q < RS_WAVES; ++q) { total += sCnt[q][tid]; before += sPart[q][tid]; }
-        }
-        unsigned x = total;
-#pragma unroll
-        for (int d = 1; d < 64; d <<= 1) {
-            const unsigned y = (unsigned)__shfl_up((int)x, d, 64);
-            if (lane >= d) x += y;
-        }
-        if (lane == 63) sScan[w] = x;
-        __syncthreads();
-#pragma unroll
-        for (int q = 0; q < RS_WAVES; ++q)
-            if (tid < 256) sCnt[q][tid] = 0u;
-        unsigned wb = 0u;
-#pragma unroll
-        for (int q = 0; q < 4; ++q) wb += (q < w) ? sScan[q] : 0u;
-        if (tid < 256) sBase[tid] = wb + x - total + before;
-        __syncthreads();
     }
     unsigned rank[RS_ROUNDS];
     volatile unsigned* myCnt = sCnt[w];
@@ -158,33 +116,38 @@
         __builtin_amdgcn_wave_barrier();
     }
     __syncthreads();
-    {
-        unsigned cnt = 0u;
-        if (tid < 256) {
-#pragma unroll
-            for (int q = 0; q < RS_WAVES; ++q) cnt += sCnt[q][tid];
-        }
-        unsigned x = cnt;
-#pragma unroll
-        for (int d = 1; d < 64; d <<= 1) {
-            const unsigned y = (unsigned)__shfl_up((int)x, d, 64);
-            if (lane >= d) x += y;
-        }
-        if (lane == 63) sScan[w] = x;
-        __syncthreads();
-        if (tid < 256) {
-            unsigned wb = 0u;
-#pragma unroll
-            for (int q = 0; q < 4; ++q) wb += (q < w) ? sScan[q] : 0u;
-            const unsigned loc = wb + x - cnt;
-            unsigned run = loc;
-#pragma unroll
-            for (int q = 0; q < RS_WAVES; ++q) {
-                const unsigned c = sCnt[q][tid];
-                sCnt[q][tid] = run;
-                run += c;
-            }
-            sBase[tid] -= loc;
+    const unsigned tag = (unsigned)(pass + 1) << 16;
+    unsigned cnt = 0u, total = 0u;
+    if (tid < 256) {
+#pragma unroll
+        for (int q = 0; q < RS_WAVES; ++q) cnt += sCnt[q][tid];
+        __hip_atomic_store(look + (size_t)tile * 256 + tid, tag | cnt, __ATOMIC_RELAXED, __HIP_MEMORY_SCOPE_AGENT);
+        total = ghist[pass * 256 + tid];
+    }
+    unsigned x = cnt, y = total;
+#pragma unroll
+    for (int d = 1; d < 64; d <<= 1) {
+        const unsigned xs = (unsigned)__shfl_up((int)x, d, 64), ys = (unsigned)__shfl_up((int)y, d, 64);
+        if (lane >= d) { x += xs; y += ys; }
+    }
+    if (lane == 63 && w < 4) { sScan[w] = x; sScan[4 + w] = y; }
+    __syncthreads();
+    unsigned delta = 0u;
+    if (tid < 256) {
+        unsigned wx = 0u, wy = 0u;
+#pragma unroll
+        for (int q = 0; q < 4; ++q) {
+            wx += (q < w) ? sScan[q] : 0u;
+            wy += (q < w) ? sScan[4 + q] : 0u;
+        }
+        const unsigned loc = wx + x - cnt;
+        delta = (wy + y - total) - loc;
+        unsigned run = loc;
+#pragma unroll
+        for (int q = 0; q < RS_WAVES; ++q) {
+            const unsigned c = sCnt[q][tid];
+            sCnt[q][tid] = run;
+            run += c;
         }
     }
     __syncthreads();
@@ -197,6 +160,47 @@
             sVal[pl] = val[r];
         }
     }
+    {
+        unsigned acc[4] = {0u, 0u, 0u, 0u};
+        const unsigned long long* rows = (const unsigned long long*)look + 2 * lane;
+        const unsigned long long empty = ((unsigned long long)tag << 32) | tag;
+        for (int k0 = w; k0 < tile; k0 += RS_LOOK * RS_WAVES) {
+            unsigned long long v[RS_LOOK][2];
+#pragma unroll
+            for (int u = 0; u < RS_LOOK; ++u) {
+                const int k = k0 + u * RS_WAVES;
+                v[u][0] = v[u][1] = empty;
+                if (k < tile) {
+                    v[u][0] = __hip_atomic_load(rows + (size_t)k * 128, __ATOMIC_RELAXED, __HIP_MEMORY_SCOPE_AGENT);
+                    v[u][1] = __hip_atomic_load(rows + (size_t)k * 128 + 1, __ATOMIC_RELAXED, __HIP_MEMORY_SCOPE_AGENT);
+                }
+            }
+#pragma unroll
+            for (int u = 0; u < RS_LOOK; ++u) {
+                for (unsigned spins = 0; !rs_row_ready(v[u], tag);) {
+                    if (++spins >= RS_SPIN_LIMIT) {
+                        atomicOr(flags, D3F_ST_OUT_OVERFLOW);
+                        v[u][0] = v[u][1] = empty;
+                        break;
+                    }
+                    __builtin_amdgcn_s_sleep(1);
+                    const size_t k = (size_t)(k0 + u * RS_WAVES);
+                    v[u][0] = __hip_atomic_load(rows + k * 128, __ATOMIC_RELAXED, __HIP_MEMORY_SCOPE_AGENT);
+                    v[u][1] = __hip_atomic_load(rows + k * 128 + 1, __ATOMIC_RELAXED, __HIP_MEMORY_SCOPE_AGENT);
+                }
+                acc[0] += (unsigned)v[u][0] & 0xffffu;
+                acc[1] += (unsigned)(v[u][0] >> 32) & 0xffffu;
+                acc[2] += (unsigned)v[u][1] & 0xffffu;
+                acc[3] += (unsigned)(v[u][1] >> 32) & 0xffffu;
+            }
+        }
+        if (tile > 0) {
+#pragma unroll
+            for (int q = 0; q < 4; ++q) atomicAdd(&sBase[4 * lane + q], acc[q]);
+        }
+    }
+    __syncthreads();
+    if (tid < 256) sBase[tid] += delta;
     __syncthreads();
     const int tile_n = min(RS_TILE, n - tile * RS_TILE);
 #pragma unroll
@@ -213,17 +217,17 @@
 #endif
 
 static inline int rs_sort_launch(const RsMeta* meta, int n_cap, unsigned* key0, unsigned* key1, unsigned* val0, unsigned* val1,
-                                 unsigned* hist, hipStream_t stream) {
+                                 unsigned* state, int* flags, hipStream_t stream) {
     const int tiles = rs_tiles(n_cap);
     static std::atomic<unsigned long long> lds_done{0ull};
     const void* const fns[] = {(const void*)rs_scatter_kernel};
     if (d3f_opt_in_lds(lds_done, fns, RS_SCATTER_LDS_BYTES) != D3F_OK) return D3F_ERR_HIP;
+    unsigned* look = state;
+    unsigned* ghist = rs_ghist(state, n_cap);
+    unsigned* tickets = ghist + RS_MAX_PASSES * 256;
     for (int p = 0; p < RS_MAX_PASSES; ++p) {
-        if (p > 0) {
-            rs_hist_kernel<<<tiles, RS_THREADS, 0, stream>>>(meta, p, key0, key1, hist);
-            D3F_LAUNCH_CHECK();
-        }
-        rs_scatter_kernel<<<tiles, RS_THREADS, RS_SCATTER_LDS_BYTES, stream>>>(meta, p, key0, key1, val0, val1, hist);
+        rs_scatter_kernel<<<tiles, RS_THREADS, RS_SCATTER_LDS_BYTES, stream>>>(meta, p, key0, key1, val0, val1, look, ghist,
+                                                                                tickets, flags);
         D3F_LAUNCH_CHECK();
     }
     return D3F_OK;
```
